# anihcsam/OpenGaussian

Hardware: AMD Instinct MI355X
Metric: fwd+bwd Mpix/s at 1080p, 1M Gaussians (RGB+6-D ins_feat); k-means it/s (higher is better)
Workload: dtype f32; 1 GPU; S1M-1080p RGB(SH3)+depth+alpha (all grads) + 6-ch ins_feat (grad to ins_feat) fwd+bwd, ONE fused 9-channel pass; gaussians=1000000, width=1920, height=1080, views_cycled=8, parallelism=single

## Files before the change

### include/ogs_raster.h

```cpp
#ifndef OGS_RASTER_H
#define OGS_RASTER_H

#include <stddef.h>
#include <stdint.h>

#ifdef __cplusplus
extern "C" {
#endif

#define OGS_OK 0
#define OGS_ERR_INVALID_ARG (-1)
#define OGS_ERR_HIP (-2)
#define OGS_ERR_UNSUPPORTED (-3)
#define OGS_ERR_SCRATCH_TOO_SMALL (-4)
#define OGS_ERR_DEVICE (-5)

#define OGS_TILE 16
#define OGS_MAX_CHANNELS 12

typedef struct OgsRasterFwdArgs {
    int32_t P;
    int32_t W, H;
    int32_t C;
    int32_t sh_degree;
    int32_t sh_coeffs;
    float tanfovx, tanfovy;
    float scale_modifier;
    int32_t prefiltered;
    int32_t debug;
    const float* bg;
    const float* means3D;
    const float* colors_precomp;
    const float* shs;
    const float* opacities;
    const float* scales;
    const float* rotations;
    const float* cov3D_precomp;
    const float* viewmatrix;
    const float* projmatrix;
    const float* campos;
    float* out_color;
    float* out_depth;
    float* out_alpha;
    int32_t* radii;
    void* geom_buffer;
    void* geom_tmp;
    void* image_buffer;
    uint32_t* point_list;
    void* binning_tmp;
    void* sorted_rec;
    void* quad_list;
    const int32_t* group_ids;
    int32_t num_groups;
    int32_t full_binning;
    void* bwd_clear;
    size_t bwd_clear_bytes;
} OgsRasterFwdArgs;

typedef struct OgsRasterBwdArgs {
    int32_t P, W, H, C, sh_degree, sh_coeffs;
    float tanfovx, tanfovy, scale_modifier;
    int32_t debug;
    int32_t num_rendered;
    int32_t geom_channels;
    const float* bg;
    const float* means3D;
    const float* colors_precomp;
    const float* shs;
    const float* opacities;
    const float* scales;
    const float* rotations;
    const float* cov3D_precomp;
    const float* viewmatrix;
    const float* projmatrix;
    const float* campos;
    const int32_t* radii;
    const float* out_alpha;
    const float* dL_dcolor;
    const float* dL_ddepth;
    const float* dL_dalpha;
    const void* geom_buffer;
    const void* image_buffer;
    const uint32_t* point_list;
    const void* sorted_rec;
    const void* quad_list;
    void* bwd_tmp;
    float* dL_dmeans2D;
    float* dL_dcolors;
    float* dL_dopacity;
    float* dL_dmeans3D;
    float* dL_dcov3D;
    float* dL_dsh;
    float* dL_dscales;
    float* dL_drotations;
    int32_t num_groups;
    float* dL_dsh_rgb;
    int32_t bwd_tmp_is_clear;
} OgsRasterBwdArgs;

int ogs_version(void);
const char* ogs_last_error(void);

int ogs_check_async_status(void);

size_t ogs_raster_geom_bytes(int32_t P, int32_t C);
size_t ogs_raster_geom_tmp_bytes(int32_t P);
size_t ogs_raster_image_bytes(int32_t W, int32_t H);
size_t ogs_raster_image_bytes_grouped(int32_t W, int32_t H, int32_t num_groups);
size_t ogs_raster_binning_tmp_bytes(int64_t num_rendered, int32_t W, int32_t H);
size_t ogs_raster_backward_tmp_bytes(int32_t P);
size_t ogs_raster_sorted_bytes(int64_t num_rendered, int32_t C);
size_t ogs_raster_quad_list_bytes(int64_t num_rendered);

int ogs_raster_forward_geometry(const OgsRasterFwdArgs* args, void* stream, int64_t* num_rendered_host);

int ogs_raster_forward_render(const OgsRasterFwdArgs* args, int64_t num_rendered, void* stream);

int ogs_raster_read_num_rendered_async(const OgsRasterFwdArgs* args, void* stream, uint32_t* host_pinned);
int ogs_raster_forward_render_deferred(const OgsRasterFwdArgs* args, int64_t capacity, void* stream);

int ogs_raster_read_num_emitted(const OgsRasterFwdArgs* args, void* stream, uint32_t* host);

size_t ogs_raster_tiny_max_points(void);
int ogs_raster_forward_tiny(const OgsRasterFwdArgs* args, void* stream);

size_t ogs_raster_tile_sort_capacity(int32_t level);

int ogs_raster_forward_reblend(const OgsRasterFwdArgs* args, void* stream);

int ogs_raster_compact_kept(int32_t W, int32_t H, int32_t C, const void* image_buffer, const void* sorted_rec,
                            const void* quad_list, void* new_image_buffer, void* new_sorted_rec, void* new_quad_list,
                            void* stream);

typedef struct OgsGroupStatsArgs {
    const int32_t* labels;
    int32_t num_labels;
    float alpha_threshold;
    float* max_alpha;
    int64_t* count;
    float* feat_sum;
    void* stats_tmp;
} OgsGroupStatsArgs;

size_t ogs_raster_stats_image_bytes(int32_t W, int32_t H, int32_t num_groups);
size_t ogs_raster_stats_tmp_bytes(int32_t num_groups, int32_t num_labels, int32_t C);
int ogs_raster_forward_group_stats(const OgsRasterFwdArgs* args, const OgsGroupStatsArgs* stats, int64_t num_rendered,
                                   void* stream);

int ogs_raster_backward(const OgsRasterBwdArgs* args, void* stream);

int ogs_mark_visible(int32_t P, const float* means3D, const float* viewmatrix, const float* projmatrix,
                     uint8_t* present, void* stream);

int ogs_sh_grad_from_views(int32_t P, int32_t V, int32_t sh_degree, int32_t sh_coeffs, const float* means3D,
                           const float* campos, const float* dL_drgb, float* dL_dsh, void* stream);

int ogs_raster_export_binning(const OgsRasterFwdArgs* args, int64_t num_rendered, uint64_t* keys_out,
                              uint32_t* ranges_out, uint32_t* n_contrib_out, void* stream);

int ogs_prof_enable(int on);
int ogs_prof_filter(const char* prefix);
int ogs_prof_collect(char* buf, size_t n);

int ogs_selftest_wave_fold16(const float* in, float* out, void* stream);
int ogs_selftest_mfma_rank1(const float* w, const float* f, const float* acc0, int32_t steps, float* out_mfma, float* out_fma,
                            void* stream);
int ogs_selftest_tile_order(const uint32_t* ranges, int64_t vtiles, uint32_t* order, void* stream);
size_t ogs_selftest_radix_tmp_bytes(int64_t n);
int ogs_selftest_radix_sort(uint32_t* keys0, uint32_t* vals0, uint32_t* keys1, uint32_t* vals1, int64_t n, int32_t key_bits,
                            int32_t variant, int32_t items, const uint32_t* n_dev, void* tmp, int32_t* result_buffer,
                            void* stream);

#ifdef __cplusplus
}
#endif
#endif
```

### opengaussian_amd/_lib.py

```python
from __future__ import annotations

import ctypes as C
import os

_HERE = os.path.dirname(os.path.abspath(__file__))
LIB_PATH = os.environ.get("OGS_LIB_PATH") or os.path.join(_HERE, "lib", "libogs_hip.so")

_f32p = C.POINTER(C.c_float)
_vp = C.c_void_p


class OgsRasterFwdArgs(C.Structure):
    _fields_ = [
        ("P", C.c_int32), ("W", C.c_int32), ("H", C.c_int32), ("C", C.c_int32),
        ("sh_degree", C.c_int32), ("sh_coeffs", C.c_int32),
        ("tanfovx", C.c_float), ("tanfovy", C.c_float), ("scale_modifier", C.c_float),
        ("prefiltered", C.c_int32), ("debug", C.c_int32),
        ("bg", _vp), ("means3D", _vp), ("colors_precomp", _vp), ("shs", _vp), ("opacities", _vp),
        ("scales", _vp), ("rotations", _vp), ("cov3D_precomp", _vp),
        ("viewmatrix", _vp), ("projmatrix", _vp), ("campos", _vp),
        ("out_color", _vp), ("out_depth", _vp), ("out_alpha", _vp), ("radii", _vp),
        ("geom_buffer", _vp), ("geom_tmp", _vp), ("image_buffer", _vp), ("point_list", _vp),
        ("binning_tmp", _vp), ("sorted_rec", _vp), ("quad_list", _vp), ("group_ids", _vp), ("num_groups", C.c_int32),
        ("full_binning", C.c_int32),
        ("bwd_clear", _vp), ("bwd_clear_bytes", C.c_size_t),
    ]


class OgsRasterBwdArgs(C.Structure):
    _fields_ = [
        ("P", C.c_int32), ("W", C.c_int32), ("H", C.c_int32), ("C", C.c_int32),
        ("sh_degree", C.c_int32), ("sh_coeffs", C.c_int32),
        ("tanfovx", C.c_float), ("tanfovy", C.c_float), ("scale_modifier", C.c_float),
        ("debug", C.c_int32), ("num_rendered", C.c_int32), ("geom_channels", C.c_int32),
        ("bg", _vp), ("means3D", _vp), ("colors_precomp", _vp), ("shs", _vp), ("opacities", _vp),
        ("scales", _vp), ("rotations", _vp), ("cov3D_precomp", _vp),
        ("viewmatrix", _vp), ("projmatrix", _vp), ("campos", _vp),
        ("radii", _vp), ("out_alpha", _vp), ("dL_dcolor", _vp), ("dL_ddepth", _vp), ("dL_dalpha", _vp),
        ("geom_buffer", _vp), ("image_buffer", _vp), ("point_list", _vp), ("sorted_rec", _vp), ("quad_list", _vp), ("bwd_tmp", _vp),
        ("dL_dmeans2D", _vp), ("dL_dcolors", _vp), ("dL_dopacity", _vp), ("dL_dmeans3D", _vp),
        ("dL_dcov3D", _vp), ("dL_dsh", _vp), ("dL_dscales", _vp), ("dL_drotations", _vp), ("num_groups", C.c_int32), ("dL_dsh_rgb", _vp),
        ("bwd_tmp_is_clear", C.c_int32),
    ]


class OgsAdamTensor(C.Structure):
    _fields_ = [("param", _vp), ("grad", _vp), ("exp_avg", _vp), ("exp_avg_sq", _vp), ("numel", C.c_int64),
                ("lr", C.c_double), ("step", C.c_int64)]


class OgsRowTensor(C.Structure):
    _fields_ = [("src", _vp), ("dst", _vp), ("width", C.c_int32), ("zero_new", C.c_int32)]


class OgsDensifyArgs(C.Structure):
    _fields_ = [("N", C.c_int32), ("grad_accum", _vp), ("denom", _vp), ("scaling", _vp), ("opacity", _vp),
                ("max_grad", C.c_float), ("min_opacity", C.c_float), ("extent", C.c_float), ("percent_dense", C.c_float),
                ("prune_world_size", C.c_int32)]


class OgsGroupStatsArgs(C.Structure):
    _fields_ = [("labels", _vp), ("num_labels", C.c_int32), ("alpha_threshold", C.c_float), ("max_alpha", _vp),
                ("count", _vp), ("feat_sum", _vp), ("stats_tmp", _vp)]


class OgsLabelMapArgs(C.Structure):
    _fields_ = [("labels", _vp), ("num_labels", C.c_int32), ("out_label", _vp), ("out_weight", _vp), ("out_second", _vp),
                ("out_alpha", _vp)]


class OgsLabelVotesArgs(C.Structure):
    _fields_ = [("pixel_labels", _vp), ("num_labels", C.c_int32), ("rows", _vp), ("num_rows", C.c_int32), ("votes", _vp)]


class OgsFeatureVotesArgs(C.Structure):
    _fields_ = [("features", _vp), ("num_channels", C.c_int32), ("valid", _vp), ("rows", _vp), ("num_rows", C.c_int32),
                ("votes", _vp)]


class OgsFeatureMapArgs(C.Structure):
    _fields_ = [("features", _vp), ("num_channels", C.c_int32), ("rows", _vp), ("num_rows", C.c_int32),
                ("channels_last", C.c_int32), ("out_map", _vp), ("out_alpha", _vp)]


class OgsRawModel(C.Structure):
    _fields_ = [("features_dc", _vp), ("features_rest", _vp), ("scaling", _vp), ("rotation", _vp), ("opacity", _vp)]


class OgsRawModelGrads(C.Structure):
    _fields_ = [("features_dc", _vp), ("features_rest", _vp), ("scaling", _vp), ("rotation", _vp), ("opacity", _vp)]


SIGNATURES = {
    "ogs_version": (C.c_int, []),
    "ogs_last_error": (C.c_char_p, []),
    "ogs_raster_geom_bytes": (C.c_size_t, [C.c_int32, C.c_int32]),
    "ogs_raster_geom_tmp_bytes": (C.c_size_t, [C.c_int32]),
    "ogs_raster_image_bytes": (C.c_size_t, [C.c_int32, C.c_int32]),
    "ogs_raster_image_bytes_grouped": (C.c_size_t, [C.c_int32, C.c_int32, C.c_int32]),
    "ogs_raster_binning_tmp_bytes": (C.c_size_t, [C.c_int64, C.c_int32, C.c_int32]),
    "ogs_raster_backward_tmp_bytes": (C.c_size_t, [C.c_int32]),
    "ogs_raster_sorted_bytes": (C.c_size_t, [C.c_int64, C.c_int32]),
    "ogs_raster_quad_list_bytes": (C.c_size_t, [C.c_int64]),
    "ogs_raster_forward_geometry": (C.c_int, [C.POINTER(OgsRasterFwdArgs), _vp, C.POINTER(C.c_int64)]),
    "ogs_raster_forward_render": (C.c_int, [C.POINTER(OgsRasterFwdArgs), C.c_int64, _vp]),
    "ogs_raster_read_num_rendered_async": (C.c_int, [C.POINTER(OgsRasterFwdArgs), _vp, _vp]),
    "ogs_raster_forward_render_deferred": (C.c_int, [C.POINTER(OgsRasterFwdArgs), C.c_int64, _vp]),
    "ogs_raster_read_num_emitted": (C.c_int, [C.POINTER(OgsRasterFwdArgs), _vp, C.POINTER(C.c_uint32)]),
    "ogs_raster_stats_image_bytes": (C.c_size_t, [C.c_int32, C.c_int32, C.c_int32]),
    "ogs_raster_stats_tmp_bytes": (C.c_size_t, [C.c_int32, C.c_int32, C.c_int32]),
    "ogs_raster_forward_group_stats": (C.c_int, [C.POINTER(OgsRasterFwdArgs), C.POINTER(OgsGroupStatsArgs), C.c_int64, _vp]),
    "ogs_raster_backward": (C.c_int, [C.POINTER(OgsRasterBwdArgs), _vp]),
    "ogs_raster_tiny_max_points": (C.c_size_t, []),
    "ogs_raster_tile_sort_capacity": (C.c_size_t, [C.c_int32]),
    "ogs_raster_forward_tiny": (C.c_int, [C.POINTER(OgsRasterFwdArgs), _vp]),
    "ogs_raster_forward_reblend": (C.c_int, [C.POINTER(OgsRasterFwdArgs), _vp]),
    "ogs_raster_compact_kept": (C.c_int, [C.c_int32, C.c_int32, C.c_int32, _vp, _vp, _vp, _vp, _vp, _vp, _vp]),
    "ogs_mark_visible": (C.c_int, [C.c_int32, _vp, _vp, _vp, _vp, _vp]),
    "ogs_sh_grad_from_views": (C.c_int, [C.c_int32, C.c_int32, C.c_int32, C.c_int32, _vp, _vp, _vp, _vp, _vp]),
    "ogs_raster_export_binning": (C.c_int, [C.POINTER(OgsRasterFwdArgs), C.c_int64, _vp, _vp, _vp, _vp]),
    "ogs_selftest_wave_fold16": (C.c_int, [_vp, _vp, _vp]),
    "ogs_selftest_mfma_rank1": (C.c_int, [_vp, _vp, _vp, C.c_int32, _vp, _vp, _vp]),
    "ogs_selftest_tile_order": (C.c_int, [_vp, C.c_int64, _vp, _vp]),
    "ogs_selftest_radix_tmp_bytes": (C.c_size_t, [C.c_int64]),
    "ogs_selftest_radix_sort": (C.c_int, [_vp, _vp, _vp, _vp, C.c_int64, C.c_int32, C.c_int32, C.c_int32, _vp, _vp, _vp, _vp]),
    "ogs_raster_forward_geometry_raw": (C.c_int, [C.POINTER(OgsRasterFwdArgs), C.POINTER(OgsRawModel), _vp,
                                                  C.POINTER(C.c_int64)]),
    "ogs_raster_forward_tiny_raw": (C.c_int, [C.POINTER(OgsRasterFwdArgs), C.POINTER(OgsRawModel), _vp]),
    "ogs_raster_backward_raw": (C.c_int, [C.POINTER(OgsRasterBwdArgs), C.POINTER(OgsRawModel), C.POINTER(OgsRawModelGrads), _vp]),
    "ogs_model_activate": (C.c_int, [C.c_int32, C.c_int32, C.POINTER(OgsRawModel), _vp, _vp, _vp, _vp, _vp]),
    "ogs_check_async_status": (C.c_int, []),
    "ogs_prof_enable": (C.c_int, [C.c_int]),
    "ogs_prof_filter": (C.c_int, [C.c_char_p]),
    "ogs_prof_collect": (C.c_int, [C.c_char_p, C.c_size_t]),
    "ogs_kmeans_tmp_bytes": (C.c_size_t, [C.c_int64, C.c_int32, C.c_int32]),
    "ogs_kmeans_lloyd": (C.c_int, [_vp, C.c_int64, C.c_int32, _vp, C.c_int32, C.c_int32, C.c_int32, C.c_int32,
                                   _vp, C.c_int64, _vp, _vp]),
    "ogs_kmeans_assign": (C.c_int, [_vp, C.c_int64, C.c_int32, _vp, C.c_int32, _vp, C.c_int64, _vp]),
    "ogs_mask_feature_sums": (C.c_int, [_vp, _vp, _vp, C.c_int32, C.c_int32, C.c_int64, C.c_int32, _vp, _vp]),
    "ogs_mask_feature_sqdev": (C.c_int, [_vp, _vp, _vp, _vp, C.c_int32, C.c_int32, C.c_int64, _vp, _vp]),
    "ogs_mask_feature_sums_backward": (C.c_int, [_vp, _vp, _vp, _vp, _vp, C.c_int32, C.c_int32, C.c_int64, _vp, _vp, _vp]),
    "ogs_mask_cohesion": (C.c_int, [_vp, _vp, _vp, C.c_int32, C.c_int32, C.c_int64, _vp, _vp]),
    "ogs_mask_cohesion_backward": (C.c_int, [_vp, _vp, _vp, _vp, C.c_int32, C.c_int32, C.c_int64, _vp, _vp, _vp]),
    "ogs_label_feature_sums": (C.c_int, [_vp, _vp, _vp, C.c_int32, C.c_int32, C.c_int64, C.c_int32, _vp, _vp]),
    "ogs_label_feature_sqdev": (C.c_int, [_vp, _vp, _vp, _vp, C.c_int32, C.c_int32, C.c_int64, _vp, _vp]),
    "ogs_label_feature_sums_backward": (C.c_int, [_vp, _vp, _vp, _vp, _vp, C.c_int32, C.c_int32, C.c_int64, _vp, _vp, _vp]),
    "ogs_label_cohesion": (C.c_int, [_vp, _vp, _vp, C.c_int32, C.c_int32, C.c_int64, _vp, _vp]),
    "ogs_label_cohesion_backward": (C.c_int, [_vp, _vp, _vp, _vp, C.c_int32, C.c_int32, C.c_int64, _vp, _vp, _vp]),
    "ogs_separation_loss": (C.c_int, [_vp, C.c_int32, C.c_int32, C.c_int32, _vp, _vp, _vp, _vp]),
    "ogs_adam_step": (C.c_int, [C.POINTER(OgsAdamTensor), C.c_int32, C.c_double, C.c_double, C.c_double, _vp]),
    "ogs_rows_gather": (C.c_int, [C.POINTER(OgsRowTensor), C.c_int32, _vp, _vp, C.c_int64, _vp]),
    "ogs_densify_tmp_bytes": (C.c_size_t, [C.c_int32]),
    "ogs_densify_plan": (C.c_int, [C.POINTER(OgsDensifyArgs), _vp, C.POINTER(C.c_uint32), _vp]),
    "ogs_densify_map": (C.c_int, [C.c_int32, _vp, _vp, _vp, _vp, _vp]),
    "ogs_densify_split_children": (C.c_int, [C.c_int64, _vp, _vp, _vp, _vp, _vp, _vp, _vp, _vp, _vp, _vp]),
    "ogs_densify_stats": (C.c_int, [C.c_int32, _vp, C.c_int32, _vp, _vp, _vp, _vp, _vp, _vp]),
    "ogs_kmeans_accumulate": (C.c_int, [_vp, C.c_int64, C.c_int32, _vp, C.c_int32, C.c_int32, _vp, _vp, _vp]),
    "ogs_kmeans_update": (C.c_int, [_vp, C.c_int32, C.c_int32, C.c_int32, _vp, _vp, _vp]),
    "ogs_kmeans_gather": (C.c_int, [_vp, _vp, C.c_int64, C.c_int32, C.c_int32, _vp, _vp]),
    "ogs_refine_wave_table_capacity": (C.c_size_t, []),
    "ogs_refine_wave_max_pixels": (C.c_size_t, []),
    "ogs_refine_block_scratch_words": (C.c_size_t, [C.c_int32]),
    "ogs_refine_visibility": (C.c_int, [C.c_int32, _vp, _vp, _vp, _vp, C.c_int32, C.c_int32, C.c_float, C.c_float, _vp,
                                        C.c_float, C.c_float, _vp, _vp]),
    "ogs_refine_footprint_labels": (C.c_int, [C.c_int32, _vp, _vp, C.c_int32, C.c_int32, C.c_int32, _vp, C.c_int32, _vp, _vp,
                                              _vp]),
    "ogs_refine_footprint_labels_block": (C.c_int, [C.c_int32, _vp, _vp, C.c_int32, C.c_int32, C.c_int32, _vp, C.c_int32, _vp,
                                                    _vp, _vp, _vp]),
    "ogs_refine_vote": (C.c_int, [C.c_int64, C.c_int32, _vp, _vp, _vp]),
    "ogs_refine_expand": (C.c_int, [C.c_int32, _vp, _vp, _vp, _vp, C.c_int32, C.c_int32, C.c_int32, _vp, C.c_int32, _vp, _vp,
                                    C.c_int32, _vp]),
    "ogs_refine_finalize": (C.c_int, [C.c_int64, C.c_int32, _vp, _vp, _vp, C.c_int32, C.c_float, _vp, _vp]),
    "ogs_loss_photometric_tmp_bytes": (C.c_size_t, [C.c_int32, C.c_int32, C.c_int32]),
    "ogs_loss_photometric_forward": (C.c_int, [_vp, _vp, C.c_int32, C.c_int32, C.c_int32, C.c_float, _vp, _vp, _vp]),
    "ogs_loss_photometric_backward": (C.c_int, [_vp, _vp, _vp, _vp, _vp, C.c_float, C.c_int32, C.c_int32, C.c_int32, _vp,
                                                _vp]),
    "ogs_loss_masked_tmp_bytes": (C.c_size_t, []),
    "ogs_loss_masked_forward": (C.c_int, [_vp, _vp, _vp, _vp, C.c_int32, C.c_int32, C.c_int32, C.c_int64, _vp, _vp, _vp]),
    "ogs_loss_masked_backward": (C.c_int, [_vp, _vp, _vp, _vp, C.c_int32, C.c_int32, C.c_int32, C.c_int64, _vp, _vp, _vp,
                                           _vp]),
    "ogs_knn_tile_points": (C.c_size_t, []),
    "ogs_knn_group_ksum": (C.c_int, [C.c_int64, _vp, C.c_int32, _vp, _vp, _vp, _vp, _vp, _vp]),
    "ogs_knn_box_points": (C.c_size_t, []),
    "ogs_knn_max_k": (C.c_size_t, []),
    "ogs_knn_neighbors_tmp_bytes": (C.c_size_t, [C.c_int64]),
    "ogs_knn_neighbors": (C.c_int, [C.c_int64, _vp, C.c_int32, C.c_int32, _vp, _vp, _vp, C.c_size_t, _vp]),
    "ogs_knn_aggregate": (C.c_int, [C.c_int64, C.c_int32, C.c_int64, C.c_int32, _vp, _vp, _vp, _vp, _vp]),
    "ogs_knn_transpose_chunk": (C.c_size_t, []),
    "ogs_knn_transpose_tmp_bytes": (C.c_size_t, [C.c_int64, C.c_int32, C.c_int64]),
    "ogs_knn_transpose": (C.c_int, [C.c_int64, C.c_int32, C.c_int64, _vp, _vp, _vp, _vp, C.c_size_t, _vp]),
    "ogs_knn_aggregate_t_tmp_bytes": (C.c_size_t, [C.c_int64, C.c_int32, C.c_int64, C.c_int32]),
    "ogs_knn_aggregate_t": (C.c_int, [C.c_int64, C.c_int32, C.c_int64, C.c_int32, _vp, _vp, _vp, _vp, _vp, _vp, C.c_size_t,
                                      _vp]),
    "ogs_knn_edge_dots": (C.c_int, [C.c_int64, C.c_int32, C.c_int64, C.c_int32, _vp, _vp, _vp, _vp, _vp]),
    "ogs_knn_smoothness_fwd_tmp_bytes": (C.c_size_t, [C.c_int64]),
    "ogs_knn_smoothness_fwd": (C.c_int, [C.c_int64, C.c_int32, C.c_int32, _vp, _vp, _vp, _vp, _vp, _vp, C.c_size_t, _vp]),
    "ogs_knn_smoothness_bwd_tmp_bytes": (C.c_size_t, [C.c_int64, C.c_int32, C.c_int32]),
    "ogs_knn_smoothness_bwd": (C.c_int, [C.c_int64, C.c_int32, C.c_int32, _vp, _vp, _vp, _vp, _vp, _vp, _vp, _vp, _vp,
                                         C.c_size_t, _vp]),
    "ogs_kmeans_wide_row_tile": (C.c_size_t, []),
    "ogs_kmeans_wide_centre_tile": (C.c_size_t, []),
    "ogs_kmeans_wide_dim_step": (C.c_size_t, []),
    "ogs_kmeans_wide_stage": (C.c_size_t, []),
    "ogs_kmeans_wide_max_dim": (C.c_size_t, []),
    "ogs_kmeans_wide_max_k": (C.c_size_t, []),
    "ogs_kmeans_wide_tmp_bytes": (C.c_size_t, [C.c_int64, C.c_int32, C.c_int32]),
    "ogs_kmeans_wide_assign": (C.c_int, [_vp, C.c_int64, C.c_int32, _vp, C.c_int32, C.c_int32, _vp, _vp, _vp, C.c_size_t, _vp]),
    "ogs_kmeans_wide_update": (C.c_int, [_vp, _vp, C.c_int64, C.c_int32, _vp, C.c_int32, C.c_int32, _vp, _vp, _vp, C.c_size_t,
                                         _vp]),
    "ogs_kmeans_wide_inertia": (C.c_int, [_vp, _vp, C.c_int64, _vp, _vp, C.c_size_t, _vp]),
    "ogs_kmeans_wide_lloyd": (C.c_int, [_vp, _vp, C.c_int64, C.c_int32, _vp, C.c_int32, C.c_int32, C.c_int32, _vp, _vp, _vp, _vp,
                                        _vp, C.c_size_t, _vp]),
    "ogs_query_max_leaves": (C.c_size_t, []),
    "ogs_query_max_top": (C.c_size_t, []),
    "ogs_query_max_classes": (C.c_size_t, []),
    "ogs_query_confusion_block": (C.c_size_t, []),
    "ogs_query_split_block": (C.c_size_t, []),
    "ogs_query_split_tmp_bytes": (C.c_size_t, [C.c_int64, C.c_int32]),
    "ogs_query_select": (C.c_int, [C.c_int32, C.c_int32, C.c_int32, _vp, _vp, _vp, _vp, C.c_int32, C.c_float, C.c_float,
                                   C.c_int32, _vp, _vp, _vp, _vp]),
    "ogs_query_classify": (C.c_int, [C.c_int64, _vp, C.c_int32, C.c_int32, _vp, _vp, _vp, _vp]),
    "ogs_query_confusion": (C.c_int, [C.c_int64, _vp, _vp, _vp, C.c_int32, _vp, _vp]),
    "ogs_query_split_count": (C.c_int, [C.c_int64, _vp, C.c_int32, _vp, _vp, C.c_int32, _vp, _vp]),
    "ogs_query_split_scan": (C.c_int, [C.c_int64, C.c_int32, _vp, _vp, _vp, _vp, _vp]),
    "ogs_query_split_scatter": (C.c_int, [C.c_int64, _vp, C.c_int32, _vp, _vp, C.c_int32, _vp, _vp, _vp, C.c_int64, _vp]),
    "ogs_raster_label_map": (C.c_int, [C.POINTER(OgsRasterFwdArgs), C.POINTER(OgsLabelMapArgs), _vp]),
    "ogs_label_map_tile_capacity": (C.c_size_t, []),
    "ogs_raster_label_votes": (C.c_int, [C.POINTER(OgsRasterFwdArgs), C.POINTER(OgsLabelVotesArgs), _vp]),
    "ogs_label_votes_quadrant_capacity": (C.c_size_t, []),
    "ogs_label_votes_fold_columns": (C.c_size_t, []),
    "ogs_raster_feature_votes": (C.c_int, [C.POINTER(OgsRasterFwdArgs), C.POINTER(OgsFeatureVotesArgs), _vp]),
    "ogs_feature_votes_fold_columns": (C.c_size_t, []),
    "ogs_feature_votes_block_columns": (C.c_size_t, []),
    "ogs_raster_feature_map": (C.c_int, [C.POINTER(OgsRasterFwdArgs), C.POINTER(OgsFeatureMapArgs), _vp]),
    "ogs_feature_map_fold_columns": (C.c_size_t, []),
    "ogs_feature_map_block_columns": (C.c_size_t, []),
}

_lib = None


class OgsError(RuntimeError):
    pass


def lib() -> C.CDLL:
    global _lib
    if _lib is None:
        if not os.path.exists(LIB_PATH):
            raise OgsError(f"{LIB_PATH} not found -- build it with `python -m opengaussian_amd.build` "
                           "(the product path has no CPU fallback)")
        import torch
        l = C.CDLL(LIB_PATH)
        for name, (res, args) in SIGNATURES.items():
            fn = getattr(l, name)
            fn.restype = res
            fn.argtypes = args
        _lib = l
    return _lib


def check(rc: int, what: str):
    if rc != 0:
        raise OgsError(f"{what} failed (code {rc}): {lib().ogs_last_error().decode()}")


def prof_filter(prefix: str):
    check(lib().ogs_prof_filter(prefix.encode()), "ogs_prof_filter")


def prof_enable(mode):
    check(lib().ogs_prof_enable(int(mode)), "ogs_prof_enable")


def prof_collect() -> dict:
    import json
    buf = C.create_string_buffer(1 << 16)
    check(lib().ogs_prof_collect(buf, len(buf)), "ogs_prof_collect")
    return json.loads(buf.value.decode())


def ptr(t):
    return None if t is None else t.data_ptr()
```

### opengaussian_amd/csrc/binning.hip

```cpp
#include <stdlib.h>
#include <string.h>

#include "ogs_common.h"

namespace ogs {

namespace {

constexpr size_t kSweepHeaderWords = 4 * 256 + 4 + 60;
constexpr int kScanItems = 8;
constexpr int kScanTile = kBlock * kScanItems;

__device__ __forceinline__ uint32_t wave_inclusive_scan(uint32_t v) {
#pragma unroll
    for (int d = 1; d < kWave; d <<= 1) {
        uint32_t t = __shfl_up(v, d, kWave);
        if (lane_id() >= d) v += t;
    }
    return v;
}

__device__ __forceinline__ uint32_t block_exclusive_scan(uint32_t v, uint32_t& total, uint32_t* wave_sums ) {
    const int wave = threadIdx.x >> 6;
    const uint32_t inc = wave_inclusive_scan(v);
    if (lane_id() == kWave - 1) wave_sums[wave] = inc;
    __syncthreads();
    uint32_t base = 0, tot = 0;
#pragma unroll
    for (int w = 0; w < kBlock / kWave; ++w) {
        const uint32_t s = wave_sums[w];
        if (w < wave) base += s;
        tot += s;
    }
    total = tot;
    __syncthreads();
    return base + inc - v;
}

__device__ __forceinline__ void load_items(const uint32_t* __restrict__ in, const uint32_t* __restrict__ gather,
                                           int64_t base, int64_t n, uint32_t item[kScanItems]) {
#pragma unroll
    for (int i = 0; i < kScanItems; ++i) {
        const int64_t idx = base + i;
        uint32_t v = 0;
        if (idx < n) v = gather ? in[gather[idx]] : in[idx];
        item[i] = v;
    }
}

__global__ __launch_bounds__(kBlock) void scan_reduce_kernel(const uint32_t* __restrict__ in,
                                                             const uint32_t* __restrict__ gather, int64_t n,
                                                             uint32_t* __restrict__ partials, const uint32_t* __restrict__ n_dev) {
    __shared__ uint32_t wave_sums[4];
    if (n_dev) n = min(n, (int64_t)*n_dev);
    const int64_t base = (int64_t)blockIdx.x * kScanTile + (int64_t)threadIdx.x * kScanItems;
    uint32_t item[kScanItems];
    load_items(in, gather, base, n, item);
    uint32_t s = 0;
#pragma unroll
    for (int i = 0; i < kScanItems; ++i) s += item[i];
    uint32_t total;
    block_exclusive_scan(s, total, wave_sums);
    if (threadIdx.x == 0) partials[blockIdx.x] = total;
}

template <bool SUM_PARTIALS>
__global__ __launch_bounds__(kBlock) void scan_apply_kernel(const uint32_t* __restrict__ in,
                                                            const uint32_t* __restrict__ gather,
                                                            uint32_t* __restrict__ out, int64_t n,
                                                            const uint32_t* __restrict__ partial_offsets,
                                                            uint32_t* __restrict__ total_out, const uint32_t* __restrict__ n_dev) {
    __shared__ uint32_t wave_sums[4];
    if (n_dev) n = min(n, (int64_t)*n_dev);
    const int64_t base = (int64_t)blockIdx.x * kScanTile + (int64_t)threadIdx.x * kScanItems;
    uint32_t item[kScanItems];
    load_items(in, gather, base, n, item);
    uint32_t s = 0;
#pragma unroll
    for (int i = 0; i < kScanItems; ++i) s += item[i];
    uint32_t block_base = 0;
    if (SUM_PARTIALS) {
        uint32_t acc = 0;
        for (uint32_t j = threadIdx.x; j < blockIdx.x; j += kBlock) acc += partial_offsets[j];
        uint32_t tot;
        block_exclusive_scan(acc, tot, wave_sums);
        block_base = tot;
    } else if (partial_offsets) {
        block_base = partial_offsets[blockIdx.x];
    }
    uint32_t total;
    uint32_t run = block_exclusive_scan(s, total, wave_sums) + block_base;
#pragma unroll
    for (int i = 0; i < kScanItems; ++i) {
        const int64_t idx = base + i;
        if (idx < n) out[idx] = run;
        run += item[i];
    }
    if (total_out && threadIdx.x == 0) {
        if (SUM_PARTIALS) { if (blockIdx.x == gridDim.x - 1) *total_out = block_base + total; }
        else if (partial_offsets == nullptr) *total_out = total;
    }
}

__global__ void scan_total_kernel(const uint32_t* __restrict__ in, const uint32_t* __restrict__ gather,
                                  const uint32_t* __restrict__ out, int64_t n, uint32_t* __restrict__ total_out,
                                  const uint32_t* __restrict__ n_dev) {
    if (threadIdx.x == 0 && blockIdx.x == 0) {
        if (n_dev) n = min(n, (int64_t)*n_dev);
        if (n <= 0) { *total_out = 0u; return; }
        const uint32_t last = gather ? in[gather[n - 1]] : in[n - 1];
        *total_out = out[n - 1] + last;
    }
}

inline int scan_blocks(int64_t n) { return (int)((n + kScanTile - 1) / kScanTile); }
constexpr int kFlatScanBlocks = 16384;

template <int ITEMS>
__global__ __launch_bounds__(kBlock) void radix_hist_kernel(const uint32_t* __restrict__ keys, int64_t n_cap,
                                                            const uint32_t* __restrict__ n_dev, int shift,
                                                            int bits, uint32_t* __restrict__ hist, int nblocks, bool drop) {
    __shared__ uint32_t h[256];
    const int64_t n = n_dev ? min((int64_t)*n_dev, n_cap) : n_cap;
    const int ndig = 1 << bits;
    const uint32_t mask = ndig - 1;
    h[threadIdx.x] = 0;
    __syncthreads();
    const int64_t base = (int64_t)blockIdx.x * (kBlock * ITEMS);
#pragma unroll
    for (int i = 0; i < ITEMS; ++i) {
        const int64_t idx = base + i * kBlock + threadIdx.x;
        if (idx < n) {
            const uint32_t k = keys[idx];
            if (!(drop && k == kDropKey)) atomicAdd(&h[(k >> shift) & mask], 1u);
        }
    }
    __syncthreads();
    if ((int)threadIdx.x < ndig) hist[(size_t)threadIdx.x * nblocks + blockIdx.x] = h[threadIdx.x];
}

__global__ __launch_bounds__(kBlock) void radix_rowscan_kernel(uint32_t* __restrict__ hist, int nblocks,
                                                               uint32_t* __restrict__ row_total) {
    __shared__ uint32_t wave_sums[4];
    uint32_t* row = hist + (size_t)blockIdx.x * nblocks;
    uint32_t carry = 0;
    for (int base = 0; base < nblocks; base += kScanTile) {
        uint32_t item[kScanItems];
        const int b0 = base + (int)threadIdx.x * kScanItems;
        uint32_t sum = 0;
#pragma unroll
        for (int i = 0; i < kScanItems; ++i) {
            item[i] = (b0 + i < nblocks) ? row[b0 + i] : 0u;
            sum += item[i];
        }
        uint32_t total;
        uint32_t run = carry + block_exclusive_scan(sum, total, wave_sums);
#pragma unroll
        for (int i = 0; i < kScanItems; ++i) {
            if (b0 + i < nblocks) row[b0 + i] = run;
            run += item[i];
        }
        carry += total;
    }
    if (threadIdx.x == 0) row_total[blockIdx.x] = carry;
}

template <int ITEMS>
__global__ __launch_bounds__(kBlock) void radix_scatter_kernel(const uint32_t* __restrict__ keys_in,
                                                               const uint32_t* __restrict__ vals_in,
                                                               uint32_t* __restrict__ keys_out,
                                                               uint32_t* __restrict__ vals_out, int64_t n_cap,
                                                               const uint32_t* __restrict__ n_dev, int shift,
                                                               int bits, const uint32_t* __restrict__ offsets,
                                                               const uint32_t* __restrict__ row_total,
                                                               int nblocks, bool drop, uint32_t* __restrict__ kept_out) {
    __shared__ uint32_t wave_hist_s[kBlock / kWave][256];
    __shared__ uint32_t scan_sums[4];
    __shared__ uint32_t dig_start[256], glob_base[256];
    __shared__ uint32_t stage_k[kBlock * ITEMS], stage_v[kBlock * ITEMS];
    volatile uint32_t(*wave_hist)[256] = wave_hist_s;
    const int64_t n = n_dev ? min((int64_t)*n_dev, n_cap) : n_cap;
    const int ndig = 1 << bits;
    const uint32_t mask = ndig - 1;
    const int tid = threadIdx.x, lane = tid & 63, wave = tid >> 6;
#pragma unroll
    for (int w = 0; w < kBlock / kWave; ++w) wave_hist_s[w][tid] = 0;
    __syncthreads();

    const int64_t base = (int64_t)blockIdx.x * (kBlock * ITEMS) + (int64_t)wave * (ITEMS * kWave);
    uint32_t key[ITEMS], val[ITEMS], rank[ITEMS];
#pragma unroll
    for (int i = 0; i < ITEMS; ++i) {
        const int64_t idx = base + i * kWave + lane;
        const bool valid = idx < n;
        key[i] = valid ? keys_in[idx] : 0xFFFFFFFFu;
        val[i] = valid ? vals_in[idx] : 0u;
    }
    const uint64_t lt_mask = (1ull << lane) - 1ull;
#pragma unroll
    for (int i = 0; i < ITEMS; ++i) {
        const int64_t idx = base + i * kWave + lane;
        const bool valid = drop ? key[i] != kDropKey : idx < n;
        const uint32_t d = (key[i] >> shift) & mask;
        uint64_t peers = __ballot(valid);
        for (int b = 0; b < bits; ++b) {
            const bool bit = (d >> b) & 1u;
            const uint64_t m = __ballot(bit);
            peers &= bit ? m : ~m;
        }
        const uint32_t r = __popcll(peers & lt_mask);
        const uint32_t cnt = __popcll(peers);
        uint32_t pre = 0;
        if (valid) pre = wave_hist[wave][d];
        __builtin_amdgcn_wave_barrier();
        if (valid && r == 0) wave_hist[wave][d] = pre + cnt;
        __builtin_amdgcn_wave_barrier();
        rank[i] = pre + r;
    }
    __syncthreads();
    uint32_t run_len = 0;
    if (tid < ndig) {
#pragma unroll
        for (int w = 0; w < kBlock / kWave; ++w) {
            const uint32_t t = wave_hist_s[w][tid];
            wave_hist_s[w][tid] = run_len;
            run_len += t;
        }
    }
    uint32_t n_valid;
    const uint32_t local_start = block_exclusive_scan(run_len, n_valid, scan_sums);
    uint32_t dummy_total;
    const uint32_t digit_base = block_exclusive_scan(tid < ndig ? row_total[tid] : 0u, dummy_total, scan_sums);
    if (kept_out != nullptr && blockIdx.x == 0 && tid == 0) *kept_out = dummy_total;
    if (tid < ndig) {
        dig_start[tid] = local_start;
        glob_base[tid] = digit_base + offsets[(size_t)tid * nblocks + blockIdx.x] - local_start;
    }
    __syncthreads();
#pragma unroll
    for (int i = 0; i < ITEMS; ++i) {
        const int64_t idx = base + i * kWave + lane;
        if (drop ? key[i] != kDropKey : idx < n) {
            const uint32_t d = (key[i] >> shift) & mask;
            const uint32_t lp = dig_start[d] + wave_hist_s[wave][d] + rank[i];
            stage_k[lp] = key[i];
            stage_v[lp] = val[i];
        }
    }
    __syncthreads();
    for (uint32_t j = tid; j < n_valid; j += kBlock) {
        const uint32_t k = stage_k[j];
        const uint32_t pos = glob_base[(k >> shift) & mask] + j;
        keys_out[pos] = k;
        vals_out[pos] = stage_v[j];
    }
}

constexpr uint32_t kStatAgg = 1u << 30, kStatInc = 2u << 30, kStatMask = (1u << 30) - 1u;
constexpr int kSpinLimit = 1 << 22;
constexpr int kLookBack = 8;
constexpr int kHistAllBlocks = 256;

struct RadixPlanDev { int npass; int shift[4]; int bits[4]; };

__global__ __launch_bounds__(kBlock) void radix_hist_all_kernel(const uint32_t* __restrict__ keys, int64_t n_cap,
                                                                const uint32_t* __restrict__ n_dev, RadixPlanDev plan,
                                                                uint32_t* __restrict__ ghist , bool drop) {
    __shared__ uint32_t h[4][256];
    const int64_t n = n_dev ? min((int64_t)*n_dev, n_cap) : n_cap;
#pragma unroll
    for (int p = 0; p < 4; ++p) h[p][threadIdx.x] = 0;
    __syncthreads();
    for (int64_t idx = (int64_t)blockIdx.x * kBlock + threadIdx.x; idx < n; idx += (int64_t)gridDim.x * kBlock) {
        const uint32_t k = keys[idx];
        if (drop && k == kDropKey) continue;
#pragma unroll
        for (int p = 0; p < 4; ++p)
            if (p < plan.npass) atomicAdd(&h[p][(k >> plan.shift[p]) & ((1u << plan.bits[p]) - 1u)], 1u);
    }
    __syncthreads();
#pragma unroll
    for (int p = 0; p < 4; ++p)
        if (p < plan.npass && h[p][threadIdx.x] != 0) atomicAdd(&ghist[p * 256 + threadIdx.x], h[p][threadIdx.x]);
}

template <int ITEMS>
__global__ __launch_bounds__(kBlock) void radix_onesweep_kernel(const uint32_t* __restrict__ keys_in,
                                                                const uint32_t* __restrict__ vals_in,
                                                                uint32_t* __restrict__ keys_out,
                                                                uint32_t* __restrict__ vals_out, int64_t n_cap,
                                                                const uint32_t* __restrict__ n_dev, int shift, int bits,
                                                                const uint32_t* __restrict__ ghist ,
                                                                uint32_t* __restrict__ status ,
                                                                uint32_t* __restrict__ ticket ,
                                                                uint32_t* __restrict__ status_word ,
                                                                int spin_limit, bool drop,
                                                                uint32_t* __restrict__ kept_out) {
    __shared__ uint32_t wave_hist_s[kBlock / kWave][256];
    __shared__ uint32_t scan_sums[4];
    __shared__ uint32_t dig_start[256], glob_base[256];
    __shared__ uint32_t stage_k[kBlock * ITEMS], stage_v[kBlock * ITEMS];
    __shared__ uint32_t s_ticket;
    volatile uint32_t(*wave_hist)[256] = wave_hist_s;
    const int64_t n = n_dev ? min((int64_t)*n_dev, n_cap) : n_cap;
    const int ndig = 1 << bits;
    const uint32_t mask = ndig - 1;
    const int tid = threadIdx.x, lane = tid & 63, wave = tid >> 6;
    if (tid == 0) s_ticket = atomicAdd(ticket, 1u);
#pragma unroll
    for (int w = 0; w < kBlock / kWave; ++w) wave_hist_s[w][tid] = 0;
    __syncthreads();
    const uint32_t tile = s_ticket;
    if ((int64_t)tile * (kBlock * ITEMS) >= n) {
        if (kept_out != nullptr && tile == 0 && tid == 0) *kept_out = 0u;
        return;
    }

    const int64_t base = (int64_t)tile * (kBlock * ITEMS) + (int64_t)wave * (ITEMS * kWave);
    uint32_t key[ITEMS], val[ITEMS], rank[ITEMS];
#pragma unroll
    for (int i = 0; i < ITEMS; ++i) {
        const int64_t idx = base + i * kWave + lane;
        const bool valid = idx < n;
        key[i] = valid ? keys_in[idx] : 0xFFFFFFFFu;
        val[i] = valid ? vals_in[idx] : 0u;
    }
    const uint64_t lt_mask = (1ull << lane) - 1ull;
#pragma unroll
    for (int i = 0; i < ITEMS; ++i) {
        const int64_t idx = base + i * kWave + lane;
        const bool valid = drop ? key[i] != kDropKey : idx < n;
        const uint32_t d = (key[i] >> shift) & mask;
        uint64_t peers = __ballot(valid);
        for (int b = 0; b < bits; ++b) {
            const bool bit = (d >> b) & 1u;
            const uint64_t m = __ballot(bit);
            peers &= bit ? m : ~m;
        }
        const uint32_t r = __popcll(peers & lt_mask);
        const uint32_t cnt = __popcll(peers);
        uint32_t pre = 0;
        if (valid) pre = wave_hist[wave][d];
        __builtin_amdgcn_wave_barrier();
        if (valid && r == 0) wave_hist[wave][d] = pre + cnt;
        __builtin_amdgcn_wave_barrier();
        rank[i] = pre + r;
    }
    __syncthreads();
    uint32_t run_len = 0;
    if (tid < ndig) {
#pragma unroll
        for (int w = 0; w < kBlock / kWave; ++w) {
            const uint32_t t = wave_hist_s[w][tid];
            wave_hist_s[w][tid] = run_len;
            run_len += t;
        }
        __hip_atomic_store(&status[(size_t)tile * 256 + tid], (tile == 0 ? kStatInc : kStatAgg) | run_len,
                           __ATOMIC_RELAXED, __HIP_MEMORY_SCOPE_AGENT);
    }
    uint32_t n_valid;
    const uint32_t local_start = block_exclusive_scan(run_len, n_valid, scan_sums);
    uint32_t dummy_total;
    const uint32_t digit_base = block_exclusive_scan(tid < ndig ? ghist[tid] : 0u, dummy_total, scan_sums);
    if (kept_out != nullptr && tile == 0 && tid == 0) *kept_out = dummy_total;
    uint32_t before = 0;
    if (tid < ndig && tile > 0) {
        int64_t pb = (int64_t)tile - 1;
        int spins = 0;
        bool done = false;
        while (!done) {
            uint32_t sw[kLookBack];
#pragma unroll
            for (int k = 0; k < kLookBack; ++k)
                sw[k] = pb - k >= 0 ? __hip_atomic_load(&status[(size_t)(pb - k) * 256 + tid], __ATOMIC_RELAXED, __HIP_MEMORY_SCOPE_AGENT)
                                    : kStatInc;
            int used = 0;
#pragma unroll
            for (int k = 0; k < kLookBack; ++k) {
                if (done || used != k) continue;
                const uint32_t flag = sw[k] & ~kStatMask;
                if (flag == 0u) continue;
                before += sw[k] & kStatMask;
                used = k + 1;
                done = flag == kStatInc;
            }
            pb -= used;
            if (!done && used < kLookBack) {
                if (++spins > spin_limit) {
                    __hip_atomic_fetch_or(status_word, kAsyncRadixSpin, __ATOMIC_RELAXED, __HIP_MEMORY_SCOPE_SYSTEM);
                    break;
                }
                __builtin_amdgcn_s_sleep(1);
            }
        }
        __hip_atomic_store(&status[(size_t)tile * 256 + tid], kStatInc | ((before + run_len) & kStatMask),
                           __ATOMIC_RELAXED, __HIP_MEMORY_SCOPE_AGENT);
    }
    if (tid < ndig) {
        dig_start[tid] = local_start;
        glob_base[tid] = digit_base + before - local_start;
    }
    __syncthreads();
#pragma unroll
    for (int i = 0; i < ITEMS; ++i) {
        const int64_t idx = base + i * kWave + lane;
        if (drop ? key[i] != kDropKey : idx < n) {
            const uint32_t d = (key[i] >> shift) & mask;
            const uint32_t lp = dig_start[d] + wave_hist_s[wave][d] + rank[i];
            stage_k[lp] = key[i];
            stage_v[lp] = val[i];
        }
    }
    __syncthreads();
    for (uint32_t j = tid; j < n_valid; j += kBlock) {
        const uint32_t k = stage_k[j];
        const uint32_t pos = glob_base[(k >> shift) & mask] + j;
        if ((int64_t)pos < n) {
            keys_out[pos] = k;
            vals_out[pos] = stage_v[j];
        }
    }
}

constexpr int kRangeItems = 4;
__global__ __launch_bounds__(kBlock) void tile_ranges_kernel(const uint32_t* __restrict__ tile_keys, int64_t D_cap,
                                                             const uint32_t* __restrict__ n_dev,
                                                             uint2* __restrict__ ranges) {
    const int64_t D = n_dev ? min((int64_t)*n_dev, D_cap) : D_cap;
    const int64_t i0 = ((int64_t)blockIdx.x * kBlock + threadIdx.x) * kRangeItems;
    if (i0 >= D) return;
    uint32_t k[kRangeItems];
    if (i0 + kRangeItems <= D) {
        const uint4 v = *reinterpret_cast<const uint4*>(tile_keys + i0);
        k[0] = v.x; k[1] = v.y; k[2] = v.z; k[3] = v.w;
    } else {
#pragma unroll
        for (int j = 0; j < kRangeItems; ++j) k[j] = i0 + j < D ? tile_keys[i0 + j] : 0u;
    }
    uint32_t prev = i0 > 0 ? tile_keys[i0 - 1] : 0u;
#pragma unroll
    for (int j = 0; j < kRangeItems; ++j) {
        const int64_t i = i0 + j;
        if (i < D) {
            const uint32_t cur = k[j];
            if (i == 0) {
                ranges[cur].x = 0;
            } else if (prev != cur) {
                ranges[prev].y = (uint32_t)i;
                ranges[cur].x = (uint32_t)i;
            }
            if (i == D - 1) ranges[cur].y = (uint32_t)D;
            prev = cur;
        }
    }
}

constexpr int kTileSortWaves = kBlock / kWave;
struct TileSortLds {
    uint32_t hist[kTileSortWaves][256];
    uint32_t dig_start[256];
    uint32_t base[256];
    uint32_t scan_sums[4];
    uint32_t red[2];
    uint2 range[kTileSortWaves];
    uint32_t kv[2 * kTileSortCap];
};
typedef __attribute__((address_space(3))) volatile uint32_t LdsWord;
typedef __attribute__((address_space(3))) unsigned long long LdsMask;
__device__ __forceinline__ LdsWord* lds_words(uint32_t* p) { return (LdsWord*)p; }
__device__ __forceinline__ LdsMask* wave_masks(TileSortLds& sm, int wave) { return (LdsMask*)(sm.kv + wave * 2 * kWaveSortCap); }

__device__ __forceinline__ void wave_rank_clear(LdsWord* hist, LdsMask* masks) {
    const int lane = threadIdx.x & (kWave - 1);
#pragma unroll
    for (int j = 0; j < 4; ++j) {
        hist[lane + j * kWave] = 0u;
        __hip_atomic_store(&masks[lane + j * kWave], 0ull, __ATOMIC_SEQ_CST, __HIP_MEMORY_SCOPE_WAVEFRONT);
    }
    __builtin_amdgcn_wave_barrier();
}

__device__ __forceinline__ void wave_rank(LdsWord* hist, LdsMask* masks, const uint32_t (&key)[kTileSortItems],
                                          uint32_t (&rank)[kTileSortItems], int ipl, int first, int m, int shift,
                                          uint32_t mask) {
    const int lane = threadIdx.x & (kWave - 1);
    const unsigned long long me = 1ull << lane;
#pragma unroll
    for (int i = 0; i < kTileSortItems; ++i) {
        if (i >= ipl) continue;
        const bool valid = first + i * kWave + lane < m;
        const uint32_t d = (key[i] >> shift) & mask;
        if (valid) __hip_atomic_fetch_or(&masks[d], me, __ATOMIC_SEQ_CST, __HIP_MEMORY_SCOPE_WAVEFRONT);
        __builtin_amdgcn_wave_barrier();
        const unsigned long long peers =
            valid ? __hip_atomic_load(&masks[d], __ATOMIC_SEQ_CST, __HIP_MEMORY_SCOPE_WAVEFRONT) : 0ull;
        const uint32_t r = __builtin_amdgcn_mbcnt_hi((uint32_t)(peers >> 32), __builtin_amdgcn_mbcnt_lo((uint32_t)peers, 0u));
        uint32_t pre = 0;
        if (valid) pre = hist[d];
        __builtin_amdgcn_wave_barrier();
        if (valid && r == 0) {
            hist[d] = pre + (uint32_t)__popcll(peers);
            __hip_atomic_store(&masks[d], 0ull, __ATOMIC_SEQ_CST, __HIP_MEMORY_SCOPE_WAVEFRONT);
        }
        __builtin_amdgcn_wave_barrier();
        rank[i] = pre + r;
    }
}

__device__ __forceinline__ void load_items(const uint32_t* __restrict__ list, const uint32_t* __restrict__ depth_keys,
                                           uint32_t (&key)[kTileSortItems], uint32_t (&val)[kTileSortItems], int ipl, int first,
                                           int m) {
#pragma unroll
    for (int i = 0; i < kTileSortItems; ++i) {
        if (i >= ipl) continue;
        val[i] = list[min(first + i * kWave, m - 1)];
    }
#pragma unroll
    for (int i = 0; i < kTileSortItems; ++i) {
        if (i >= ipl) continue;
        key[i] = depth_keys[val[i] & kGidMask];
    }
}

__device__ __forceinline__ uint32_t tile_sort_rank(TileSortLds& sm, const uint32_t (&key)[kTileSortItems],
                                                   uint32_t (&rank)[kTileSortItems], int ipl, int chunk, int m, int shift,
                                                   uint32_t mask) {
    const int tid = threadIdx.x, wave = tid >> 6;
    LdsWord* hist = lds_words(sm.hist[wave]);
    LdsMask* masks = wave_masks(sm, wave);
    wave_rank_clear(hist, masks);
    wave_rank(hist, masks, key, rank, ipl, wave * chunk, m, shift, mask);
    __syncthreads();
    uint32_t run_len = 0;
#pragma unroll
    for (int w = 0; w < kTileSortWaves; ++w) {
        const uint32_t t = sm.hist[w][tid];
        sm.hist[w][tid] = run_len;
        run_len += t;
    }
    uint32_t total;
    sm.dig_start[tid] = block_exclusive_scan(run_len, total, sm.scan_sums);
    __syncthreads();
    return run_len;
}

__device__ __forceinline__ void wave_sort_list(TileSortLds& sm, uint32_t* __restrict__ seg, int n,
                                               const uint32_t* __restrict__ depth_keys) {
    const int lane = threadIdx.x & (kWave - 1), wave = threadIdx.x >> 6;
    LdsWord* wk = lds_words(sm.kv + wave * 2 * kWaveSortCap);
    LdsWord* wv = wk + kWaveSortCap;
    LdsWord* hist = lds_words(sm.hist[wave]);
    LdsMask* masks = wave_masks(sm, wave);
    uint32_t key[kTileSortItems], val[kTileSortItems], rank[kTileSortItems];
    const int ipl = (n + kWave - 1) / kWave;
    load_items(seg, depth_keys, key, val, ipl, lane, n);
    uint32_t k_and = 0xFFFFFFFFu, k_or = 0u;
#pragma unroll
    for (int i = 0; i < kTileSortItems; ++i) {
        if (i >= ipl) continue;
        k_and &= key[i];
        k_or |= key[i];
    }
#pragma unroll
    for (int d = 32; d >= 1; d >>= 1) {
        k_and &= (uint32_t)__shfl_xor((int)k_and, d, kWave);
        k_or |= (uint32_t)__shfl_xor((int)k_or, d, kWave);
    }
    const uint32_t diff = (uint32_t)__builtin_amdgcn_readfirstlane((int)(k_and ^ k_or));
    if (diff == 0u) return;
    const int lo = __builtin_ctz(diff), hi = 31 - __builtin_clz(diff);
    const int npass = (hi - lo + 8) / 8;
    const int per = (hi - lo + npass) / npass;
    for (int p = 0; p < npass; ++p) {
        const int shift = lo + p * per, bits = min(per, hi + 1 - shift);
        const uint32_t mask = (1u << bits) - 1u;
        wave_rank_clear(hist, masks);
        wave_rank(hist, masks, key, rank, ipl, 0, n, shift, mask);
        uint32_t c[4], sum = 0;
#pragma unroll
        for (int j = 0; j < 4; ++j) { c[j] = hist[4 * lane + j]; sum += c[j]; }
        uint32_t run = wave_inclusive_scan(sum) - sum;
#pragma unroll
        for (int j = 0; j < 4; ++j) { hist[4 * lane + j] = run; run += c[j]; }
        __builtin_amdgcn_wave_barrier();
#pragma unroll
        for (int i = 0; i < kTileSortItems; ++i) {
            if (i >= ipl) continue;
            rank[i] += hist[(key[i] >> shift) & mask];
        }
#pragma unroll
        for (int i = 0; i < kTileSortItems; ++i) {
            if (i >= ipl) continue;
            if (i * kWave + lane < n) {
                wk[rank[i]] = key[i];
                wv[rank[i]] = val[i];
            }
        }
        __builtin_amdgcn_wave_barrier();
        if (p + 1 < npass) {
#pragma unroll
            for (int i = 0; i < kTileSortItems; ++i) {
                if (i >= ipl) continue;
                const int e = min(i * kWave + lane, n - 1);
                key[i] = wk[e];
                val[i] = wv[e];
            }
            __builtin_amdgcn_wave_barrier();
        }
    }
    for (int j = lane; j < n; j += kWave) seg[j] = wv[j];
}

__device__ __forceinline__ void block_sort_list(TileSortLds& sm, uint32_t* __restrict__ seg, uint32_t* __restrict__ alt, int n,
                                                const uint32_t* __restrict__ depth_keys) {
    const int tid = threadIdx.x, lane = tid & 63, wave = tid >> 6;
    const bool in_lds = n <= kTileSortCap;
    uint32_t key[kTileSortItems], val[kTileSortItems], rank[kTileSortItems];
    __syncthreads();
    if (tid < 2) sm.red[tid] = tid == 0 ? 0xFFFFFFFFu : 0u;
    uint32_t k_and = 0xFFFFFFFFu, k_or = 0u;
    const int ipl0 = (min(n, kTileSortCap) + kBlock - 1) / kBlock, chunk0 = ipl0 * kWave;
    if (in_lds) {
        load_items(seg, depth_keys, key, val, ipl0, wave * chunk0 + lane, n);
#pragma unroll
        for (int i = 0; i < kTileSortItems; ++i) {
            if (i >= ipl0) continue;
            k_and &= key[i];
            k_or |= key[i];
        }
    } else {
        for (int j = tid; j < n; j += kBlock) {
            const uint32_t k = depth_keys[seg[j] & kGidMask];
            k_and &= k;
            k_or |= k;
        }
    }
#pragma unroll
    for (int d = 32; d >= 1; d >>= 1) {
        k_and &= (uint32_t)__shfl_xor((int)k_and, d, kWave);
        k_or |= (uint32_t)__shfl_xor((int)k_or, d, kWave);
    }
    __syncthreads();
    if (lane == 0) { atomicAnd(&sm.red[0], k_and); atomicOr(&sm.red[1], k_or); }
    __syncthreads();
    const uint32_t diff = sm.red[0] ^ sm.red[1];
    if (diff == 0u) return;
    const int lo = __builtin_ctz(diff), hi = 31 - __builtin_clz(diff);
    const int npass = (hi - lo + 8) / 8;
    const int per = (hi - lo + npass) / npass;
    uint32_t* const sk = sm.kv;
    uint32_t* const sv = sm.kv + kTileSortCap;

    if (in_lds) {
        for (int p = 0; p < npass; ++p) {
            const int shift = lo + p * per, bits = min(per, hi + 1 - shift);
            const uint32_t mask = (1u << bits) - 1u;
            tile_sort_rank(sm, key, rank, ipl0, chunk0, n, shift, mask);
#pragma unroll
            for (int i = 0; i < kTileSortItems; ++i) {
                if (i >= ipl0) continue;
                const uint32_t d = (key[i] >> shift) & mask;
                rank[i] += sm.dig_start[d] + sm.hist[wave][d];
            }
#pragma unroll
            for (int i = 0; i < kTileSortItems; ++i) {
                if (i >= ipl0) continue;
                if (wave * chunk0 + i * kWave + lane < n) {
                    sk[rank[i]] = key[i];
                    sv[rank[i]] = val[i];
                }
            }
            __syncthreads();
            if (p + 1 < npass) {
#pragma unroll
                for (int i = 0; i < kTileSortItems; ++i) {
                    if (i >= ipl0) continue;
                    const int e = min(wave * chunk0 + i * kWave + lane, n - 1);
                    key[i] = sk[e];
                    val[i] = sv[e];
                }
                __syncthreads();
            }
        }
        for (int j = tid; j < n; j += kBlock) seg[j] = sv[j];
        return;
    }

    for (int p = 0; p < npass; ++p) {
        const int shift = lo + p * per, bits = min(per, hi + 1 - shift);
        const uint32_t mask = (1u << bits) - 1u;
        const uint32_t* __restrict__ src = (p & 1) ? alt : seg;
        uint32_t* __restrict__ dst = (p & 1) ? seg : alt;
        sm.base[tid] = 0u;
        __syncthreads();
        for (int j = tid; j < n; j += kBlock) atomicAdd(&sm.base[(depth_keys[src[j] & kGidMask] >> shift) & mask], 1u);
        __syncthreads();
        uint32_t total;
        const uint32_t start = block_exclusive_scan(sm.base[tid], total, sm.scan_sums);
        sm.base[tid] = start;
        for (int c0 = 0; c0 < n; c0 += kTileSortCap) {
            const int m = min(kTileSortCap, n - c0);
            const int ipl = (m + kBlock - 1) / kBlock, chunk = ipl * kWave;
            load_items(src + c0, depth_keys, key, val, ipl, wave * chunk + lane, m);
            const uint32_t cnt = tile_sort_rank(sm, key, rank, ipl, chunk, m, shift, mask);
#pragma unroll
            for (int i = 0; i < kTileSortItems; ++i) {
                if (i >= ipl) continue;
                if (wave * chunk + i * kWave + lane < m) {
                    const uint32_t d = (key[i] >> shift) & mask;
                    dst[sm.base[d] + sm.hist[wave][d] + rank[i]] = val[i];
                }
            }
            __syncthreads();
            sm.base[tid] += cnt;
        }
        __syncthreads();
    }
    if (npass & 1) {
        for (int j = tid; j < n; j += kBlock) seg[j] = alt[j];
    }
}

__global__ __launch_bounds__(kBlock) void tile_depth_sort_kernel(const uint2* __restrict__ ranges, int tiles,
                                                                 const uint32_t* __restrict__ tile_order,
                                                                 uint32_t* __restrict__ point_list,
                                                                 const uint32_t* __restrict__ depth_keys,
                                                                 uint32_t* __restrict__ scratch) {
    __shared__ TileSortLds sm;
    const int wave = threadIdx.x >> 6;
    if (threadIdx.x < kTileSortWaves) {
        const int b = blockIdx.x * kTileSortWaves + threadIdx.x;
        sm.range[threadIdx.x] = b < tiles ? ranges[tile_order ? tile_order[b] : (uint32_t)b] : make_uint2(0u, 0u);
    }
    __syncthreads();
    const uint32_t x = (uint32_t)__builtin_amdgcn_readfirstlane((int)sm.range[wave].x);
    const int n = __builtin_amdgcn_readfirstlane((int)(sm.range[wave].y - sm.range[wave].x));
    if (n >= 2 && n <= kWaveSortCap) wave_sort_list(sm, point_list + x, n, depth_keys);
#pragma unroll 1
    for (int w = 0; w < kTileSortWaves; ++w) {
        const uint32_t xw = (uint32_t)__builtin_amdgcn_readfirstlane((int)sm.range[w].x);
        const int nw = __builtin_amdgcn_readfirstlane((int)(sm.range[w].y - sm.range[w].x));
        if (nw > kWaveSortCap) block_sort_list(sm, point_list + xw, scratch + xw, nw, depth_keys);
    }
}

__global__ __launch_bounds__(kBlock) void export_keys_kernel(const uint2* __restrict__ ranges,
                                                             const uint32_t* __restrict__ point_list,
                                                             const float4* __restrict__ rec, int recv4,
                                                             uint64_t* __restrict__ keys_out) {
    const uint32_t tile = blockIdx.x;
    const uint2 r = ranges[tile];
    for (uint32_t i = r.x + threadIdx.x; i < r.y; i += kBlock) {
        const uint32_t gid = point_list[i] & kGidMask;
        const uint32_t bits = __float_as_uint(rec[(size_t)gid * recv4].z);
        keys_out[i] = ((uint64_t)tile << 32) | bits;
    }
}

}

size_t scan_tmp_bytes(int64_t n) {
    size_t total = 0;
    int64_t m = n;
    while (true) {
        const int nb = scan_blocks(m);
        if (nb <= 1) break;
        total += align_up((size_t)nb * sizeof(uint32_t));
        m = nb;
    }
    return total + kAlign;
}

size_t sort_tmp_bytes(int64_t n) {
    const int64_t hist = (int64_t)256 * sort_blocks_for(n > 0 ? n : 1);
    const size_t legacy = align_up((size_t)hist * sizeof(uint32_t)) + align_up(256 * sizeof(uint32_t)) + scan_tmp_bytes(hist);
    const int64_t tiles4 = ((n > 0 ? n : 1) + kBlock * 4 - 1) / (kBlock * 4);
    const size_t sweep = align_up(kSweepHeaderWords * sizeof(uint32_t)) + 4 * align_up((size_t)256 * tiles4 * sizeof(uint32_t));
    return legacy > sweep ? legacy : sweep;
}

static int sweep_items_for(int64_t n, int forced) {
    if (forced == 4 || forced == 16) return forced;
    return n <= (int64_t)(256 << 10) ? 4 : 16;
}

bool radix_onesweep_enabled(int64_t n) {
    static const int forced = [] {
        const char* e = getenv("OGS_RADIX");
        return !e ? 0 : strcmp(e, "legacy") == 0 ? 1 : strcmp(e, "sweep") == 0 ? 2 : 0;
    }();
    if (forced == 1 || n >= (int64_t)kStatMask) return false;
    return forced == 2 || n <= (int64_t)(256 << 10);
}

namespace {
struct SweepTmp {
    uint32_t* ghist;
    uint32_t* ticket;
    uint32_t* status[4];
    size_t zero_bytes;
    static SweepTmp carve(void* tmp, int64_t n, int npass, int items_forced) {
        SweepTmp t;
        char* p = static_cast<char*>(tmp);
        t.ghist = reinterpret_cast<uint32_t*>(p);
        t.ticket = t.ghist + 4 * 256;
        const int items = sweep_items_for(n, items_forced);
        const int64_t tiles = ((n > 0 ? n : 1) + (int64_t)kBlock * items - 1) / ((int64_t)kBlock * items);
        const size_t table = align_up((size_t)256 * tiles * sizeof(uint32_t));
        char* q = p + align_up(kSweepHeaderWords * sizeof(uint32_t));
        for (int i = 0; i < 4; ++i) t.status[i] = reinterpret_cast<uint32_t*>(q + (size_t)i * table);
        t.zero_bytes = align_up(kSweepHeaderWords * sizeof(uint32_t)) + (size_t)npass * table;
        return t;
    }
};
}

int radix_sort_begin(const uint32_t* keys, int64_t n, const uint32_t* n_dev, int npass, const int* shifts, const int* bits,
                     void* tmp, hipStream_t stream, int debug, bool drop, int items) {
    if (n <= 0) return OGS_OK;
    if (npass < 1 || npass > 4) { set_error("radix_sort_begin: npass=%d out of range", npass); return OGS_ERR_INVALID_ARG; }
    const SweepTmp t = SweepTmp::carve(tmp, n, npass, items);
    OGS_HIP_CHECK(hipMemsetAsync(tmp, 0, t.zero_bytes, stream));
    RadixPlanDev plan{};
    plan.npass = npass;
    for (int i = 0; i < npass; ++i) {
        if (bits[i] < 1 || bits[i] > 8) { set_error("radix_sort_begin: bits=%d out of range", bits[i]); return OGS_ERR_INVALID_ARG; }
        plan.shift[i] = shifts[i];
        plan.bits[i] = bits[i];
    }
    const int64_t want = (n + kBlock * 16 - 1) / (kBlock * 16);
    const int grid = (int)(want < 1 ? 1 : (want > kHistAllBlocks ? kHistAllBlocks : want));
    OGS_LAUNCH(radix_hist_all_kernel, dim3(grid), dim3(kBlock), 0, stream, keys, n, n_dev, plan, t.ghist, drop);
    OGS_LAUNCH_CHECK(debug, stream);
    return OGS_OK;
}

int radix_sort_pass(int pass, int npass, const uint32_t* keys_in, const uint32_t* vals_in, uint32_t* keys_out, uint32_t* vals_out,
                    int64_t n, int shift, int bits, void* tmp, hipStream_t stream, int debug, const uint32_t* n_dev, bool drop,
                    uint32_t* kept_out, int items_forced, int spin_limit) {
    if (n <= 0) return OGS_OK;
    const SweepTmp t = SweepTmp::carve(tmp, n, npass, items_forced);
    const int items = sweep_items_for(n, items_forced);
    const int nb = (int)((n + (int64_t)kBlock * items - 1) / ((int64_t)kBlock * items));
    uint32_t* status_word = async_status_word();
    if (!status_word) return OGS_ERR_HIP;
    if (spin_limit < 0) spin_limit = kSpinLimit;
    if (items == 4) {
        OGS_LAUNCH(radix_onesweep_kernel<4>, dim3(nb), dim3(kBlock), 0, stream, keys_in, vals_in, keys_out, vals_out, n, n_dev,
                   shift, bits, (const uint32_t*)(t.ghist + pass * 256), t.status[pass], t.ticket + pass, status_word, spin_limit,
                   drop, kept_out);
    } else {
        OGS_LAUNCH(radix_onesweep_kernel<16>, dim3(nb), dim3(kBlock), 0, stream, keys_in, vals_in, keys_out, vals_out, n, n_dev,
                   shift, bits, (const uint32_t*)(t.ghist + pass * 256), t.status[pass], t.ticket + pass, status_word, spin_limit,
                   drop, kept_out);
    }
    OGS_LAUNCH_CHECK(debug, stream);
    return OGS_OK;
}

int exclusive_scan_u32(const uint32_t* in, const uint32_t* gather, uint32_t* out, int64_t n, uint32_t* total,
                       void* tmp, hipStream_t stream, int debug, const uint32_t* n_dev) {
    if (n <= 0) {
        if (total) OGS_HIP_CHECK(hipMemsetAsync(total, 0, sizeof(uint32_t), stream));
        return OGS_OK;
    }
    const int nb = scan_blocks(n);
    if (nb == 1) {
        OGS_LAUNCH(scan_apply_kernel<false>, dim3(1), dim3(kBlock), 0, stream, in, gather, out, n,
                           (const uint32_t*)nullptr, total, n_dev);
        OGS_LAUNCH_CHECK(debug, stream);
        return OGS_OK;
    }
    uint32_t* partials = static_cast<uint32_t*>(tmp);
    void* next_tmp = static_cast<char*>(tmp) + align_up((size_t)nb * sizeof(uint32_t));
    OGS_LAUNCH(scan_reduce_kernel, dim3(nb), dim3(kBlock), 0, stream, in, gather, n, partials, n_dev);
    OGS_LAUNCH_CHECK(debug, stream);
    if (nb <= kFlatScanBlocks) {
        OGS_LAUNCH(scan_apply_kernel<true>, dim3(nb), dim3(kBlock), 0, stream, in, gather, out, n,
                           (const uint32_t*)partials, total, n_dev);
        OGS_LAUNCH_CHECK(debug, stream);
        return OGS_OK;
    }
    int rc = exclusive_scan_u32(partials, nullptr, partials, nb, nullptr, next_tmp, stream, debug, nullptr);
    if (rc != OGS_OK) return rc;
    OGS_LAUNCH(scan_apply_kernel<false>, dim3(nb), dim3(kBlock), 0, stream, in, gather, out, n,
                       (const uint32_t*)partials, (uint32_t*)nullptr, n_dev);
    OGS_LAUNCH_CHECK(debug, stream);
    if (total) {
        if (in == out) { set_error("exclusive_scan_u32: total with in-place scan unsupported"); return OGS_ERR_INVALID_ARG; }
        OGS_LAUNCH(scan_total_kernel, dim3(1), dim3(64), 0, stream, in, gather, (const uint32_t*)out, n, total, n_dev);
        OGS_LAUNCH_CHECK(debug, stream);
    }
    return OGS_OK;
}

int radix_pass(const uint32_t* keys_in, const uint32_t* vals_in, uint32_t* keys_out, uint32_t* vals_out, int64_t n,
               int shift, int bits, void* tmp, hipStream_t stream, int debug, const uint32_t* n_dev, bool drop,
               uint32_t* kept_out) {
    if (n <= 0) return OGS_OK;
    if (bits < 1 || bits > 8) { set_error("radix_pass: bits=%d out of range", bits); return OGS_ERR_INVALID_ARG; }
    const int items = sort_items_for(n);
    const int nb = sort_blocks_for(n);
    const int ndig = 1 << bits;
    uint32_t* hist = static_cast<uint32_t*>(tmp);
    uint32_t* row_total = reinterpret_cast<uint32_t*>(static_cast<char*>(tmp) + align_up((size_t)256 * nb * sizeof(uint32_t)));
    if (items == 4) {
        OGS_LAUNCH(radix_hist_kernel<4>, dim3(nb), dim3(kBlock), 0, stream, keys_in, n, n_dev, shift, bits, hist, nb, drop);
    } else {
        OGS_LAUNCH(radix_hist_kernel<8>, dim3(nb), dim3(kBlock), 0, stream, keys_in, n, n_dev, shift, bits, hist, nb, drop);
    }
    OGS_LAUNCH_CHECK(debug, stream);
    OGS_LAUNCH(radix_rowscan_kernel, dim3(ndig), dim3(kBlock), 0, stream, hist, nb, row_total);
    OGS_LAUNCH_CHECK(debug, stream);
    if (items == 4) {
        OGS_LAUNCH(radix_scatter_kernel<4>, dim3(nb), dim3(kBlock), 0, stream, keys_in, vals_in, keys_out, vals_out, n, n_dev,
                   shift, bits, (const uint32_t*)hist, (const uint32_t*)row_total, nb, drop, kept_out);
    } else {
        OGS_LAUNCH(radix_scatter_kernel<8>, dim3(nb), dim3(kBlock), 0, stream, keys_in, vals_in, keys_out, vals_out, n, n_dev,
                   shift, bits, (const uint32_t*)hist, (const uint32_t*)row_total, nb, drop, kept_out);
    }
    OGS_LAUNCH_CHECK(debug, stream);
    return OGS_OK;
}

int launch_tile_ranges(const uint32_t* tile_keys_sorted, int64_t D, uint2* ranges, int64_t tiles, hipStream_t s,
                       int debug, const uint32_t* n_dev, bool already_zeroed) {
    if (!already_zeroed) OGS_HIP_CHECK(hipMemsetAsync(ranges, 0, (size_t)tiles * sizeof(uint2), s));
    if (D <= 0) return OGS_OK;
    const int grid = (int)((D + (int64_t)kBlock * kRangeItems - 1) / ((int64_t)kBlock * kRangeItems));
    OGS_LAUNCH(tile_ranges_kernel, dim3(grid), dim3(kBlock), 0, s, tile_keys_sorted, D, n_dev, ranges);
    OGS_LAUNCH_CHECK(debug, s);
    return OGS_OK;
}

int launch_tile_depth_sort(const uint2* ranges, int64_t tiles, const uint32_t* tile_order, uint32_t* point_list,
                           const uint32_t* depth_keys, uint32_t* scratch, hipStream_t s, int debug) {
    if (tiles <= 0) return OGS_OK;
    if (tiles >= (1ll << 31)) { set_error("tile_depth_sort: %lld tiles", (long long)tiles); return OGS_ERR_UNSUPPORTED; }
    const unsigned grid = (unsigned)((tiles + kTileSortWaves - 1) / kTileSortWaves);
    OGS_LAUNCH(tile_depth_sort_kernel, dim3(grid), dim3(kBlock), 0, s, ranges, (int)tiles, tile_order, point_list, depth_keys,
               scratch);
    OGS_LAUNCH_CHECK(debug, s);
    return OGS_OK;
}

int launch_export_keys(const uint2* ranges, int tiles, const uint32_t* point_list, const float4* rec, int recv4,
                       uint64_t* keys_out, hipStream_t s) {
    OGS_LAUNCH(export_keys_kernel, dim3(tiles), dim3(kBlock), 0, s, ranges, point_list, rec, recv4, keys_out);
    OGS_LAUNCH_CHECK(0, s);
    return OGS_OK;
}

}
```

### opengaussian_amd/csrc/capi.hip

```cpp
#include <stdarg.h>
#include <stdlib.h>
#include <string.h>

#include <map>
#include <mutex>
#include <string>
#include <vector>

#include "ogs_common.h"

namespace ogs {

static thread_local char g_err[512] = "";

void set_error(const char* fmt, ...) {
    va_list ap;
    va_start(ap, fmt);
    vsnprintf(g_err, sizeof(g_err), fmt, ap);
    va_end(ap);
}

namespace {
struct ProfRec { const char* name; hipEvent_t start, stop; };
int g_prof_mode = 0;
char g_prof_prefix[64] = "blend_";
std::vector<ProfRec> g_prof;
std::vector<hipEvent_t> g_event_pool;
std::mutex g_prof_mu;
hipEvent_t take_event() {
    if (!g_event_pool.empty()) { hipEvent_t e = g_event_pool.back(); g_event_pool.pop_back(); return e; }
    hipEvent_t e = nullptr;
    (void)hipEventCreate(&e);
    return e;
}
}

ProfScope::ProfScope(const char* n, hipStream_t s) : name(n), stream(s), slot(-1) {
    if (g_prof_mode == 0) return;
    if (g_prof_mode == 2 && strncmp(n, g_prof_prefix, strlen(g_prof_prefix)) != 0) return;
    std::lock_guard<std::mutex> lk(g_prof_mu);
    ProfRec r{n, take_event(), take_event()};
    (void)hipEventRecord(r.start, s);
    g_prof.push_back(r);
    slot = (int)g_prof.size() - 1;
}
ProfScope::~ProfScope() {
    if (slot < 0) return;
    std::lock_guard<std::mutex> lk(g_prof_mu);
    (void)hipEventRecord(g_prof[slot].stop, stream);
}

namespace {
uint32_t* g_async_status = nullptr;
std::mutex g_async_mu;
}
uint32_t* async_status_word() {
    std::lock_guard<std::mutex> lk(g_async_mu);
    if (!g_async_status) {
        void* p = nullptr;
        const hipError_t e = hipHostMalloc(&p, 64, hipHostMallocMapped | hipHostMallocPortable);
        if (e != hipSuccess || !p) {
            set_error("hipHostMalloc of the async status word failed: %s", hipGetErrorString(e));
            return nullptr;
        }
        memset(p, 0, 64);
        g_async_status = static_cast<uint32_t*>(p);
    }
    return g_async_status;
}
int take_async_status() {
    std::lock_guard<std::mutex> lk(g_async_mu);
    if (!g_async_status) return 0;
    return (int)__atomic_exchange_n(g_async_status, 0u, __ATOMIC_ACQ_REL);
}
int check_async_status(const char* where) {
    const int st = take_async_status();
    if (st == 0) return OGS_OK;
    set_error("%s: a kernel of an earlier launch reported status 0x%x%s%s -- the results of the passes since the last check "
              "are not valid", where, st,
              (st & (int)kAsyncRadixSpin) ? " (one-launch radix pass: a look-back wait exceeded its bound)" : "",
              (st & (int)kAsyncSplitOverflow) ? " (query split: the scatter met more rows than its capacity)" : "");
    return OGS_ERR_DEVICE;
}

}
int ogs::blend_prefetch_lines() {
    static const int v = [] {
        const char* e = getenv("OGS_BLEND_PREFETCH");
        const int n = e ? atoi(e) : kPrefetchMax;
        const int lines = (n & 0xFF) > kPrefetchMax ? kPrefetchMax : (n & 0xFF);
#ifdef OGS_EXPERIMENTS
        return n < 0 ? 0 : (lines | (n & 0x300));
#else
        return n < 0 ? 0 : lines;
#endif
    }();
    return v;
}
namespace ogs {

static int bit_length(uint32_t v) {
    int n = 0;
    while (v) { ++n; v >>= 1; }
    return n;
}

static int validate_fwd(const OgsRasterFwdArgs* a, bool images = true) {
    if (!a) { set_error("args == NULL"); return OGS_ERR_INVALID_ARG; }
    if (a->P < 0 || a->W <= 0 || a->H <= 0) { set_error("bad sizes P=%d W=%d H=%d", a->P, a->W, a->H); return OGS_ERR_INVALID_ARG; }
    if (a->C != 3 && a->C != 6 && a->C != 9 && a->C != 12) { set_error("C=%d unsupported (3, 6, 9, 12)", a->C); return OGS_ERR_UNSUPPORTED; }
    if (a->shs == nullptr && a->colors_precomp == nullptr) {
        set_error("provide shs or colors_precomp"); return OGS_ERR_INVALID_ARG;
    }
    if (a->shs != nullptr && (a->colors_precomp != nullptr) != (a->C > 3)) {
        set_error("with shs: C == 3 and no colors_precomp, or C > 3 with colors_precomp holding the C-3 extra channels");
        return OGS_ERR_INVALID_ARG;
    }
    const bool sr = a->scales != nullptr && a->rotations != nullptr;
    if (sr == (a->cov3D_precomp != nullptr) || (a->scales != nullptr) != (a->rotations != nullptr)) {
        set_error("provide exactly one of (scales, rotations) / cov3D_precomp"); return OGS_ERR_INVALID_ARG;
    }
    if (a->shs) {
        if (a->sh_degree < 0 || a->sh_degree > 3 || a->sh_coeffs < (a->sh_degree + 1) * (a->sh_degree + 1)) {
            set_error("sh_degree=%d needs >= %d coefficients, got %d", a->sh_degree, (a->sh_degree + 1) * (a->sh_degree + 1), a->sh_coeffs);
            return OGS_ERR_INVALID_ARG;
        }
    }
    if (!a->bg || !a->viewmatrix || !a->projmatrix || !a->campos || (images && (!a->out_color || !a->out_depth || !a->out_alpha))) {
        set_error("NULL required pointer"); return OGS_ERR_INVALID_ARG;
    }
    if (a->P > 0 && (!a->means3D || !a->opacities || !a->radii || !a->geom_buffer || !a->geom_tmp)) {
        set_error("NULL required per-Gaussian pointer"); return OGS_ERR_INVALID_ARG;
    }
    if (a->num_groups < 0 || (a->num_groups > 1 && a->P > 0 && !a->group_ids)) {
        set_error("num_groups=%d needs group_ids", a->num_groups); return OGS_ERR_INVALID_ARG;
    }
    return OGS_OK;
}

static int validate_raw(const OgsRawModel* raw, int P, int M) {
    if (!raw) { set_error("raw == NULL"); return OGS_ERR_INVALID_ARG; }
    if (M < 1) { set_error("raw model: sh_coeffs=%d < 1", M); return OGS_ERR_INVALID_ARG; }
    if (P > 0 && (!raw->features_dc || !raw->scaling || !raw->rotation || !raw->opacity)) {
        set_error("raw model: NULL features_dc / scaling / rotation / opacity"); return OGS_ERR_INVALID_ARG;
    }
    if (P > 0 && M > 1 && !raw->features_rest) { set_error("raw model: features_rest == NULL with %d SH coefficients", M); return OGS_ERR_INVALID_ARG; }
    return OGS_OK;
}

static int raw_fwd_args(const OgsRasterFwdArgs* a, const OgsRawModel* raw, OgsRasterFwdArgs* out) {
    if (!a) { set_error("args == NULL"); return OGS_ERR_INVALID_ARG; }
    if (a->shs || a->opacities || a->scales || a->rotations || a->cov3D_precomp) {
        set_error("raw pass: args.shs / opacities / scales / rotations / cov3D_precomp must be NULL (the raw model takes their place)");
        return OGS_ERR_INVALID_ARG;
    }
    int rc = validate_raw(raw, a->P, a->sh_coeffs);
    if (rc != OGS_OK) return rc;
    *out = *a;
    out->shs = raw->features_dc;
    out->opacities = raw->opacity;
    out->scales = raw->scaling;
    out->rotations = raw->rotation;
    if (a->P == 0) {
        out->shs = out->scales = out->rotations = a->bg;
    }
    return OGS_OK;
}

}

using namespace ogs;

extern "C" {

int ogs_version(void) { return 408; }

int ogs_check_async_status(void) { return check_async_status("ogs_check_async_status"); }

int ogs_prof_enable(int on) {
    std::lock_guard<std::mutex> lk(g_prof_mu);
    for (auto& r : g_prof) { g_event_pool.push_back(r.start); g_event_pool.push_back(r.stop); }
    g_prof.clear();
    g_prof_mode = on;
    return OGS_OK;
}

int ogs_prof_filter(const char* prefix) {
    std::lock_guard<std::mutex> lk(g_prof_mu);
    if (!prefix || strlen(prefix) >= sizeof(g_prof_prefix)) { set_error("prof_filter: prefix NULL or longer than %zu", sizeof(g_prof_prefix) - 1); return OGS_ERR_INVALID_ARG; }
    strcpy(g_prof_prefix, prefix);
    return OGS_OK;
}

int ogs_prof_collect(char* buf, size_t n) {
    std::lock_guard<std::mutex> lk(g_prof_mu);
    std::map<std::string, std::pair<long, double>> agg;
    for (auto& r : g_prof) {
        OGS_HIP_CHECK(hipEventSynchronize(r.stop));
        float ms = 0.f;
        OGS_HIP_CHECK(hipEventElapsedTime(&ms, r.start, r.stop));
        auto& a = agg[r.name];
        a.first += 1;
        a.second += ms;
    }
    std::string out = "{";
    bool first = true;
    for (auto& kv : agg) {
        char line[384];
        std::string nm = kv.first;
        for (auto& ch : nm) if (ch == '"') ch = '\'';
        snprintf(line, sizeof(line), "%s\"%s\": {\"calls\": %ld, \"total_ms\": %.6f}", first ? "" : ", ", nm.c_str(),
                 kv.second.first, kv.second.second);
        out += line;
        first = false;
    }
    out += "}";
    if (!buf || out.size() + 1 > n) { set_error("prof_collect: buffer too small (%zu needed)", out.size() + 1); return OGS_ERR_SCRATCH_TOO_SMALL; }
    memcpy(buf, out.c_str(), out.size() + 1);
    return OGS_OK;
}
const char* ogs_last_error(void) { return g_err; }

size_t ogs_raster_geom_bytes(int32_t P, int32_t C) { return GeomState::bytes(P > 0 ? P : 1, C); }
size_t ogs_raster_geom_tmp_bytes(int32_t P) { return GeomTmp::bytes(P > 0 ? P : 1); }
size_t ogs_raster_image_bytes(int32_t W, int32_t H) { return ImageState::bytes(W, H); }
size_t ogs_raster_image_bytes_grouped(int32_t W, int32_t H, int32_t G) { return ImageState::bytes(W, H, num_groups_of(G)); }
size_t ogs_raster_binning_tmp_bytes(int64_t D, int32_t, int32_t) { return BinTmp::bytes(D > 0 ? D : 1); }
size_t ogs_raster_sorted_bytes(int64_t D, int32_t C) {
    return align_up((size_t)(D > 0 ? D : 1) * stream_vec4(C) * sizeof(float4));
}
size_t ogs_raster_quad_list_bytes(int64_t D) {
    return align_up((size_t)(5 * (D > 0 ? D : 1) + 2 * kQuadPad) * sizeof(uint32_t));
}
size_t ogs_raster_backward_tmp_bytes(int32_t P) { return align_up((size_t)(P > 0 ? P : 1) * 16 * sizeof(double)); }

static int forward_geometry_impl(const OgsRasterFwdArgs* a_in, void* stream_, int64_t* num_rendered_host, bool raw,
                                 const float* raw_rest) {
    int rc = validate_fwd(a_in, false);
    if (rc != OGS_OK) return rc;
    OgsRasterFwdArgs a_raw;
    const OgsRasterFwdArgs* a = a_in;
    if (raw) { a_raw = *a_in; a_raw.cov3D_precomp = raw_rest; a = &a_raw; }
    hipStream_t s = static_cast<hipStream_t>(stream_);
    if (num_rendered_host) *num_rendered_host = 0;
    if (a->P == 0) return OGS_OK;
    rc = check_async_status("forward (entry)");
    if (rc != OGS_OK) return rc;
    const GeomState gs = GeomState::carve(a->geom_buffer, a->P, a->C);
    const GeomTmp gt = GeomTmp::carve(a->geom_tmp, a->P);
    if (a->P <= kSmallMaxP) {
        rc = launch_small_geometry(*a, gs, gt, s, raw);
        if (rc != OGS_OK) return rc;
    } else if (per_tile_depth_order(*a)) {
        rc = launch_preprocess(*a, gs, gt, s, raw);
        if (rc != OGS_OK) return rc;
        rc = block_sum_offsets(*a) ? launch_block_offsets(*a, gt, s)
                                   : exclusive_scan_u32(gt.tiles_touched, nullptr, gt.offsets, a->P, gt.num_rendered, gt.sort_tmp, s, a->debug);
        if (rc != OGS_OK) return rc;
    } else {
        rc = launch_preprocess(*a, gs, gt, s, raw);
        if (rc != OGS_OK) return rc;
        const bool sweep = radix_onesweep_enabled(a->P);
        if (sweep) {
            const int shifts[4] = {0, 8, 16, 24}, nbits[4] = {8, 8, 8, 8};
            rc = radix_sort_begin(gt.keys[0], a->P, nullptr, 4, shifts, nbits, gt.sort_tmp, s, a->debug, true);
            if (rc != OGS_OK) return rc;
        }
        for (int pass = 0; pass < 4; ++pass) {
            const int in = pass & 1, out = in ^ 1;
            const bool drop = pass == 0;
            const uint32_t* n_pass = drop ? nullptr : gt.visible();
            rc = sweep ? radix_sort_pass(pass, 4, gt.keys[in], gt.order[in], gt.keys[out], gt.order[out], a->P, 8 * pass, 8, gt.sort_tmp, s, a->debug, n_pass, drop, drop ? gt.visible() : nullptr)
                       : radix_pass(gt.keys[in], gt.order[in], gt.keys[out], gt.order[out], a->P, 8 * pass, 8, gt.sort_tmp, s, a->debug, n_pass, drop, drop ? gt.visible() : nullptr);
            if (rc != OGS_OK) return rc;
        }
        rc = exclusive_scan_u32(gt.tiles_touched, gt.order[0], gt.offsets, a->P, gt.num_rendered, gt.sort_tmp, s, a->debug, gt.visible());
        if (rc != OGS_OK) return rc;
    }
    if (num_rendered_host) {
        uint32_t d = 0;
        OGS_HIP_CHECK(hipMemcpyAsync(&d, gt.num_rendered, sizeof(uint32_t), hipMemcpyDeviceToHost, s));
        OGS_HIP_CHECK(hipStreamSynchronize(s));
        *num_rendered_host = (int64_t)d;
        rc = check_async_status("forward geometry phase");
        if (rc != OGS_OK) return rc;
    }
    return OGS_OK;
}

int ogs_raster_forward_geometry(const OgsRasterFwdArgs* a, void* stream_, int64_t* num_rendered_host) {
    return forward_geometry_impl(a, stream_, num_rendered_host, false, nullptr);
}

int ogs_raster_forward_geometry_raw(const OgsRasterFwdArgs* a, const OgsRawModel* raw, void* stream_, int64_t* num_rendered_host) {
    OgsRasterFwdArgs b;
    const int rc = raw_fwd_args(a, raw, &b);
    if (rc != OGS_OK) return rc;
    return forward_geometry_impl(&b, stream_, num_rendered_host, true, raw->features_rest);
}

int ogs_model_activate(int32_t P, int32_t M, const OgsRawModel* raw, float* scales, float* rotations, float* opacities, float* shs,
                       void* stream_) {
    if (P < 0) { set_error("model_activate: P=%d", P); return OGS_ERR_INVALID_ARG; }
    if (P == 0) return OGS_OK;
    if (!raw) { set_error("model_activate: raw == NULL"); return OGS_ERR_INVALID_ARG; }
    if ((scales && !raw->scaling) || (rotations && !raw->rotation) || (opacities && !raw->opacity) ||
        (shs && (M < 1 || !raw->features_dc || (M > 1 && !raw->features_rest)))) {
        set_error("model_activate: an output is requested whose raw input is NULL (M=%d)", M); return OGS_ERR_INVALID_ARG;
    }
    return launch_model_activate(P, M, *raw, scales, rotations, opacities, shs, static_cast<hipStream_t>(stream_));
}

int ogs_raster_read_num_rendered_async(const OgsRasterFwdArgs* a, void* stream_, uint32_t* host_pinned) {
    if (!a || !host_pinned) { set_error("read_num_rendered_async: NULL pointer"); return OGS_ERR_INVALID_ARG; }
    if (a->P == 0) { *host_pinned = 0; return OGS_OK; }
    const GeomTmp gt = GeomTmp::carve(a->geom_tmp, a->P);
    OGS_HIP_CHECK(hipMemcpyAsync(host_pinned, gt.num_rendered, sizeof(uint32_t), hipMemcpyDeviceToHost,
                                 static_cast<hipStream_t>(stream_)));
    return OGS_OK;
}

int ogs_raster_read_num_emitted(const OgsRasterFwdArgs* a, void* stream_, uint32_t* host) {
    if (!a || !host) { set_error("read_num_emitted: NULL pointer"); return OGS_ERR_INVALID_ARG; }
    *host = 0;
    if (a->P == 0) return OGS_OK;
    if (!a->geom_tmp) { set_error("read_num_emitted: geom_tmp == NULL"); return OGS_ERR_INVALID_ARG; }
    const GeomTmp gt = GeomTmp::carve(a->geom_tmp, a->P);
    hipStream_t s = static_cast<hipStream_t>(stream_);
    OGS_HIP_CHECK(hipMemcpyAsync(host, block_sum_offsets(*a) ? gt.emitted() : gt.num_rendered, sizeof(uint32_t), hipMemcpyDeviceToHost, s));
    OGS_HIP_CHECK(hipStreamSynchronize(s));
    return OGS_OK;
}

static int render_impl(const OgsRasterFwdArgs* a, int64_t D, bool deferred, hipStream_t s,
                       const OgsGroupStatsArgs* stats = nullptr) {
    int rc = validate_fwd(a, stats == nullptr);
    if (rc != OGS_OK) return rc;
    if (!a->image_buffer) { set_error("image_buffer == NULL"); return OGS_ERR_INVALID_ARG; }
    if (a->bwd_clear && !stats && (((uintptr_t)a->bwd_clear | a->bwd_clear_bytes) & 15u) != 0) {
        set_error("bwd_clear / bwd_clear_bytes must be multiples of 16"); return OGS_ERR_INVALID_ARG;
    }
    const int G = num_groups_of(a->num_groups);
    const ImageState is = stats ? ImageState::carve_stats(a->image_buffer, a->W, a->H, G)
                                : ImageState::carve(a->image_buffer, a->W, a->H, G);
    const int gx = (a->W + kTile - 1) / kTile, gy = (a->H + kTile - 1) / kTile;
    const int64_t tiles = (int64_t)gx * gy * G;
    if (tiles >= (1ll << 31)) { set_error("%d groups x %d tiles exceed 2^31 virtual tiles", G, gx * gy); return OGS_ERR_UNSUPPORTED; }
    const GeomState gs = GeomState::carve(a->geom_buffer, a->P > 0 ? a->P : 1, a->C);
    const bool per_tile = per_tile_depth_order(*a);
    bool order_ready = false;
    if (D > 0) {
        if (!a->point_list || !a->binning_tmp) { set_error("point_list / binning_tmp == NULL with num_rendered=%lld", (long long)D); return OGS_ERR_INVALID_ARG; }
        if (D >= (1ll << 31)) { set_error("num_rendered=%lld exceeds 2^31", (long long)D); return OGS_ERR_UNSUPPORTED; }
        const GeomTmp gt = GeomTmp::carve(a->geom_tmp, a->P);
        const BinTmp bt = BinTmp::carve(a->binning_tmp, D);
        const int bits = bit_length((uint32_t)(tiles - 1));
        const int passes = bits == 0 ? 1 : (bits + 7) / 8;
        const int per = bits == 0 ? 1 : (bits + passes - 1) / passes;
        uint32_t* vbuf[2];
        vbuf[passes & 1] = a->point_list;
        vbuf[(passes & 1) ^ 1] = bt.vals;
        const uint32_t* n_dev = block_sum_offsets(*a) ? gt.emitted() : deferred ? gt.num_rendered : nullptr;
        const bool cull = a->full_binning == 0;
        const bool zero_in_dup = tiles <= (int64_t)a->P;
        rc = launch_duplicate(*a, gs, gt, bt.tile_keys[0], vbuf[0], (uint32_t)D, cull, !per_tile, s,
                              zero_in_dup ? is.ranges : nullptr, zero_in_dup ? (int)tiles : 0);
        if (rc != OGS_OK) return rc;
        const bool sweep = radix_onesweep_enabled(D);
        int shifts[4], nbits[4];
        for (int p = 0; p < passes; ++p) {
            shifts[p] = p * per;
            nbits[p] = (p == passes - 1) ? (bits == 0 ? 1 : bits - shifts[p]) : per;
        }
        if (passes == 2 && (bits & 1)) {
            nbits[0] = bits / 2; shifts[1] = nbits[0]; nbits[1] = bits - nbits[0];
        }
        if (sweep) {
            rc = radix_sort_begin(bt.tile_keys[0], D, n_dev, passes, shifts, nbits, bt.sort_tmp, s, a->debug, cull);
            if (rc != OGS_OK) return rc;
        }
        for (int p = 0; p < passes; ++p) {
            const int in = p & 1, out = in ^ 1;
            const bool drop = cull && p == 0;
            const uint32_t* n_pass = (cull && p > 0) ? bt.kept : n_dev;
            rc = sweep ? radix_sort_pass(p, passes, bt.tile_keys[in], vbuf[in], bt.tile_keys[out], vbuf[out], D, shifts[p], nbits[p], bt.sort_tmp, s, a->debug, n_pass, drop, drop ? bt.kept : nullptr)
                       : radix_pass(bt.tile_keys[in], vbuf[in], bt.tile_keys[out], vbuf[out], D, shifts[p], nbits[p], bt.sort_tmp, s, a->debug, n_pass, drop, drop ? bt.kept : nullptr);
            if (rc != OGS_OK) return rc;
        }
        rc = launch_tile_ranges(bt.tile_keys[passes & 1], D, is.ranges, tiles, s, a->debug, cull ? bt.kept : n_dev, zero_in_dup);
        if (rc != OGS_OK) return rc;
        if (per_tile) {
            const uint32_t* order = launch_tile_order(is, tiles, a->P, s, a->debug);
            order_ready = true;
            rc = launch_tile_depth_sort(is.ranges, tiles, order, a->point_list, gt.keys[0], bt.vals, s, a->debug);
            if (rc != OGS_OK) return rc;
        }
    } else {
        OGS_HIP_CHECK(hipMemsetAsync(is.ranges, 0, (size_t)tiles * sizeof(uint2), s));
    }
    if (stats) return launch_group_stats(*a, *stats, gs, is, s, order_ready);
    if (!a->sorted_rec || !a->quad_list) { set_error("sorted_rec / quad_list == NULL"); return OGS_ERR_INVALID_ARG; }
    return launch_blend_forward(*a, gs, is, D, s, order_ready);
}

int ogs_raster_forward_render(const OgsRasterFwdArgs* a, int64_t D, void* stream_) {
    return render_impl(a, D, false, static_cast<hipStream_t>(stream_));
}

size_t ogs_raster_stats_image_bytes(int32_t W, int32_t H, int32_t G) {
    return ImageState::stats_bytes(W > 0 ? W : 1, H > 0 ? H : 1, num_groups_of(G));
}
size_t ogs_raster_stats_tmp_bytes(int32_t G, int32_t L, int32_t C) {
    return align_up((size_t)num_groups_of(G) * (size_t)((L > 0 ? L : 0) + 1) * (size_t)(C > 0 ? C : 1) * sizeof(int64_t));
}

int ogs_raster_forward_group_stats(const OgsRasterFwdArgs* a, const OgsGroupStatsArgs* st, int64_t D, void* stream_) {
    if (!a || !st) { set_error("forward_group_stats: NULL argument"); return OGS_ERR_INVALID_ARG; }
    if (st->num_labels < 0) { set_error("forward_group_stats: num_labels=%d < 0", st->num_labels); return OGS_ERR_INVALID_ARG; }
    if (!st->labels || !st->max_alpha || !st->count || !st->feat_sum || !st->stats_tmp) {
        set_error("forward_group_stats: NULL labels / output / stats_tmp pointer"); return OGS_ERR_INVALID_ARG;
    }
    if (D < 0) { set_error("forward_group_stats: num_rendered=%lld < 0", (long long)D); return OGS_ERR_INVALID_ARG; }
    if (a->P == 0) D = 0;
    return render_impl(a, D, false, static_cast<hipStream_t>(stream_), st);
}

int ogs_raster_forward_render_deferred(const OgsRasterFwdArgs* a, int64_t capacity, void* stream_) {
    if (capacity <= 0) { set_error("forward_render_deferred: capacity must be > 0"); return OGS_ERR_INVALID_ARG; }
    return render_impl(a, capacity, true, static_cast<hipStream_t>(stream_));
}

int ogs_raster_forward_reblend(const OgsRasterFwdArgs* a, void* stream_) {
    if (!a) { set_error("args == NULL"); return OGS_ERR_INVALID_ARG; }
    if (a->P <= 0 || a->W <= 0 || a->H <= 0) { set_error("forward_reblend: bad sizes P=%d W=%d H=%d", a->P, a->W, a->H); return OGS_ERR_INVALID_ARG; }
    if (a->C != 3 && a->C != 6 && a->C != 9 && a->C != 12) { set_error("C=%d unsupported (3, 6, 9, 12)", a->C); return OGS_ERR_UNSUPPORTED; }
    if (a->num_groups > 1) { set_error("forward_reblend: grouped passes are not kept"); return OGS_ERR_UNSUPPORTED; }
    if (!a->colors_precomp || !a->bg || !a->out_color || !a->out_depth || !a->out_alpha || !a->image_buffer || !a->sorted_rec ||
        !a->quad_list) {
        set_error("forward_reblend: NULL required pointer (colors_precomp, bg, out_*, image_buffer, sorted_rec, quad_list)");
        return OGS_ERR_INVALID_ARG;
    }
    const int rc = check_async_status("forward_reblend (entry)");
    if (rc != OGS_OK) return rc;
    const ImageState is = ImageState::carve(a->image_buffer, a->W, a->H, 1);
    return launch_reblend(*a, is, static_cast<hipStream_t>(stream_));
}

int ogs_raster_compact_kept(int32_t W, int32_t H, int32_t C, const void* image_buffer, const void* sorted_rec, const void* quad_list,
                            void* new_image_buffer, void* new_sorted_rec, void* new_quad_list, void* stream_) {
    if (W <= 0 || H <= 0) { set_error("compact_kept: bad sizes W=%d H=%d", W, H); return OGS_ERR_INVALID_ARG; }
    if (!image_buffer || !sorted_rec || !quad_list || !new_image_buffer || !new_sorted_rec || !new_quad_list) {
        set_error("compact_kept: NULL pointer"); return OGS_ERR_INVALID_ARG;
    }
    const ImageState is_old = ImageState::carve(const_cast<void*>(image_buffer), W, H, 1);
    const ImageState is_new = ImageState::carve(new_image_buffer, W, H, 1);
    return launch_compact_kept(W, H, C, is_old, is_new, sorted_rec, quad_list, new_sorted_rec, new_quad_list,
                               static_cast<hipStream_t>(stream_));
}

size_t ogs_raster_tiny_max_points(void) { return (size_t)kTinyMaxP; }

size_t ogs_raster_tile_sort_capacity(int32_t level) {
    return level == 0 ? (size_t)kWaveSortCap : level == 1 ? (size_t)kTileSortCap : 0;
}

static int forward_tiny_impl(const OgsRasterFwdArgs* a_in, void* stream_, bool raw, const float* raw_rest) {
    int rc = validate_fwd(a_in);
    if (rc != OGS_OK) return rc;
    OgsRasterFwdArgs a_raw;
    const OgsRasterFwdArgs* a = a_in;
    if (raw) { a_raw = *a_in; a_raw.cov3D_precomp = raw_rest; a = &a_raw; }
    if (a->P <= 0 || a->P > kTinyMaxP) { set_error("forward_tiny: P=%d outside [1, %d]", a->P, kTinyMaxP); return OGS_ERR_INVALID_ARG; }
    if (a->num_groups > 1) { set_error("forward_tiny: grouped passes use the streaming path"); return OGS_ERR_UNSUPPORTED; }
    hipStream_t s = static_cast<hipStream_t>(stream_);
    const GeomState gs = GeomState::carve(a->geom_buffer, a->P, a->C);
    uint32_t* order = static_cast<uint32_t*>(a->geom_tmp);
    rc = launch_tiny_geometry(*a, gs, order, s, raw);
    if (rc != OGS_OK) return rc;
    return launch_tiny_blend(*a, gs, order, s);
}

int ogs_raster_forward_tiny(const OgsRasterFwdArgs* a, void* stream_) { return forward_tiny_impl(a, stream_, false, nullptr); }

int ogs_raster_forward_tiny_raw(const OgsRasterFwdArgs* a, const OgsRawModel* raw, void* stream_) {
    OgsRasterFwdArgs b;
    const int rc = raw_fwd_args(a, raw, &b);
    if (rc != OGS_OK) return rc;
    return forward_tiny_impl(&b, stream_, true, raw->features_rest);
}

static int backward_impl(const OgsRasterBwdArgs* a, void* stream_, const OgsRawModelGrads* raw_grads) {
    if (!a) { set_error("args == NULL"); return OGS_ERR_INVALID_ARG; }
    if (a->C != 3 && a->C != 6 && a->C != 9) { set_error("backward: C=%d unsupported (3, 6, 9)", a->C); return OGS_ERR_UNSUPPORTED; }
    if (a->P == 0) return OGS_OK;
    const bool feat_only = backward_is_features_only(*a);
    if (!a->dL_dcolor || !a->image_buffer || !a->bwd_tmp || !a->radii) {
        set_error("backward: NULL required pointer"); return OGS_ERR_INVALID_ARG;
    }
    if (!feat_only && (!a->geom_buffer || !a->bg || !a->means3D || !a->viewmatrix || !a->projmatrix || !a->campos)) {
        set_error("backward: NULL required pointer"); return OGS_ERR_INVALID_ARG;
    }
    if (!feat_only && a->num_rendered > 0 && !a->point_list) { set_error("backward: point_list == NULL"); return OGS_ERR_INVALID_ARG; }
    if ((int64_t)a->P * grad_stride(a->C) >= (1ll << 32)) {
        set_error("backward: P=%d exceeds the %lld Gaussians the 32-bit gradient-record offsets address", a->P,
                  (long long)((1ll << 32) / grad_stride(a->C)) - 1);
        return OGS_ERR_UNSUPPORTED;
    }
    {
        const int st = check_async_status("backward (entry)");
        if (st != OGS_OK) return st;
    }
    hipStream_t s = static_cast<hipStream_t>(stream_);
    const GeomState gs = GeomState::carve(const_cast<void*>(a->geom_buffer), a->P, a->C);
    if (a->num_groups < 0) { set_error("backward: num_groups=%d", a->num_groups); return OGS_ERR_INVALID_ARG; }
    const ImageState is = ImageState::carve(const_cast<void*>(a->image_buffer), a->W, a->H, num_groups_of(a->num_groups));
    void* grad_rec = a->bwd_tmp;
    const int rec_doubles = feat_only ? feat_grad_stride(a->C, a->shs ? 3 : 0) : grad_stride(a->C);
    if (!a->bwd_tmp_is_clear) OGS_HIP_CHECK(hipMemsetAsync(grad_rec, 0, (size_t)a->P * rec_doubles * sizeof(double), s));
    if (a->num_rendered > 0 && (!a->sorted_rec || !a->quad_list)) { set_error("backward: sorted_rec / quad_list == NULL"); return OGS_ERR_INVALID_ARG; }
    int rc = launch_blend_backward(*a, is, grad_rec, s);
    if (rc != OGS_OK) return rc;
    return launch_preprocess_backward(*a, gs, grad_rec, s, raw_grads);
}

int ogs_raster_backward(const OgsRasterBwdArgs* a, void* stream_) { return backward_impl(a, stream_, nullptr); }

int ogs_raster_backward_raw(const OgsRasterBwdArgs* a, const OgsRawModel* raw, const OgsRawModelGrads* grads, void* stream_) {
    if (!a) { set_error("args == NULL"); return OGS_ERR_INVALID_ARG; }
    if (a->shs || a->opacities || a->scales || a->rotations || a->cov3D_precomp || a->dL_dsh || a->dL_dopacity || a->dL_dscales ||
        a->dL_drotations || a->dL_dcov3D) {
        set_error("raw backward: args.shs / opacities / scales / rotations / cov3D_precomp and their dL_d* outputs must be NULL "
                  "(the raw model and its gradient struct take their place)");
        return OGS_ERR_INVALID_ARG;
    }
    const int rc = validate_raw(raw, a->P, a->sh_coeffs);
    if (rc != OGS_OK) return rc;
    static const OgsRawModelGrads kNoGrads = {nullptr, nullptr, nullptr, nullptr, nullptr};
    const OgsRawModelGrads* g = grads ? grads : &kNoGrads;
    if (g->features_rest && !raw->features_rest) { set_error("raw backward: a features_rest gradient without features_rest"); return OGS_ERR_INVALID_ARG; }
    OgsRasterBwdArgs b = *a;
    b.shs = raw->features_dc;
    b.opacities = raw->opacity;
    b.scales = raw->scaling;
    b.rotations = raw->rotation;
    b.cov3D_precomp = raw->features_rest;
    b.dL_dsh = g->features_dc ? g->features_dc : g->features_rest;
    b.dL_dopacity = g->opacity;
    b.dL_dscales = g->scaling;
    b.dL_drotations = g->rotation;
    return backward_impl(&b, stream_, g);
}

int ogs_mark_visible(int32_t P, const float* means3D, const float* viewmatrix, const float*, uint8_t* present,
                     void* stream_) {
    if (P == 0) return OGS_OK;
    if (!means3D || !viewmatrix || !present) { set_error("mark_visible: NULL pointer"); return OGS_ERR_INVALID_ARG; }
    return launch_mark_visible(P, means3D, viewmatrix, present, static_cast<hipStream_t>(stream_));
}

int ogs_sh_grad_from_views(int32_t P, int32_t V, int32_t sh_degree, int32_t sh_coeffs, const float* means3D,
                           const float* campos, const float* dL_drgb, float* dL_dsh, void* stream_) {
    if (P == 0) return OGS_OK;
    if (P < 0 || V < 1 || sh_degree < 0 || sh_degree > 3 || sh_coeffs < (sh_degree + 1) * (sh_degree + 1)) {
        set_error("sh_grad_from_views: bad sizes P=%d V=%d degree=%d coeffs=%d", P, V, sh_degree, sh_coeffs);
        return OGS_ERR_INVALID_ARG;
    }
    if (!means3D || !campos || !dL_drgb || !dL_dsh) { set_error("sh_grad_from_views: NULL pointer"); return OGS_ERR_INVALID_ARG; }
    return launch_sh_grad_from_views(P, V, sh_degree, sh_coeffs, means3D, campos, dL_drgb, dL_dsh,
                                     static_cast<hipStream_t>(stream_));
}

int ogs_selftest_wave_fold16(const float* in, float* out, void* stream_) {
    if (!in || !out) { set_error("selftest: NULL pointer"); return OGS_ERR_INVALID_ARG; }
    return launch_wave_fold16_test(in, out, static_cast<hipStream_t>(stream_));
}

int ogs_selftest_mfma_rank1(const float* w, const float* f, const float* acc0, int32_t steps, float* out_mfma, float* out_fma,
                            void* stream_) {
    if (!w || !f || !acc0 || !out_mfma || !out_fma || steps < 0) { set_error("selftest: NULL pointer / steps < 0"); return OGS_ERR_INVALID_ARG; }
    return launch_mfma_rank1_test(w, f, acc0, steps, out_mfma, out_fma, static_cast<hipStream_t>(stream_));
}

int ogs_selftest_tile_order(const uint32_t* ranges, int64_t vtiles, uint32_t* order, void* stream_) {
    if (!ranges || !order || vtiles <= 0) { set_error("selftest: NULL pointer / no tiles"); return OGS_ERR_INVALID_ARG; }
    return launch_tile_order_test(ranges, vtiles, order, static_cast<hipStream_t>(stream_));
}

size_t ogs_selftest_radix_tmp_bytes(int64_t n) { return sort_tmp_bytes(n > 0 ? n : 1); }

int ogs_selftest_radix_sort(uint32_t* keys0, uint32_t* vals0, uint32_t* keys1, uint32_t* vals1, int64_t n, int32_t key_bits,
                            int32_t variant, int32_t items, const uint32_t* n_dev, void* tmp, int32_t* result_buffer,
                            void* stream_) {
    if (!result_buffer) { set_error("selftest_radix_sort: NULL result_buffer"); return OGS_ERR_INVALID_ARG; }
    *result_buffer = 0;
    if (n <= 0) return OGS_OK;
    if (items != 0 && items != 4 && items != 16) { set_error("selftest_radix_sort: items=%d (0, 4 or 16)", items); return OGS_ERR_INVALID_ARG; }
    if (!keys0 || !vals0 || !keys1 || !vals1 || !tmp || key_bits < 1 || key_bits > 32) {
        set_error("selftest_radix_sort: bad arguments"); return OGS_ERR_INVALID_ARG;
    }
    hipStream_t s = static_cast<hipStream_t>(stream_);
    uint32_t* k[2] = {keys0, keys1};
    uint32_t* v[2] = {vals0, vals1};
    const int passes = (key_bits + 7) / 8, per = (key_bits + passes - 1) / passes;
    int shifts[4], nbits[4];
    for (int p = 0; p < passes; ++p) { shifts[p] = p * per; nbits[p] = p == passes - 1 ? key_bits - shifts[p] : per; }
    const bool sweep = (variant & 1) != 0, drop = (variant & 2) != 0;
    const int spin_limit = (variant & 4) ? 0 : -1;
    (void)take_async_status();
    uint32_t* kept = nullptr;
    if (drop) {
        OGS_HIP_CHECK(hipMalloc(&kept, sizeof(uint32_t)));
        OGS_HIP_CHECK(hipMemsetAsync(kept, 0xA5, sizeof(uint32_t), s));
    }
    int rc = OGS_OK;
    if (sweep) rc = radix_sort_begin(k[0], n, n_dev, passes, shifts, nbits, tmp, s, 0, drop, items);
    for (int p = 0; p < passes && rc == OGS_OK; ++p) {
        const int in = p & 1, out = in ^ 1;
        const bool d0 = drop && p == 0;
        const uint32_t* n_pass = (drop && p > 0) ? kept : n_dev;
        rc = sweep ? radix_sort_pass(p, passes, k[in], v[in], k[out], v[out], n, shifts[p], nbits[p], tmp, s, 0, n_pass, d0, d0 ? kept : nullptr, items, spin_limit)
                   : radix_pass(k[in], v[in], k[out], v[out], n, shifts[p], nbits[p], tmp, s, 0, n_pass, d0, d0 ? kept : nullptr);
    }
    uint32_t kept_host = 0;
    if (drop) {
        if (rc == OGS_OK && hipMemcpyAsync(&kept_host, kept, sizeof(uint32_t), hipMemcpyDeviceToHost, s) != hipSuccess) rc = OGS_ERR_HIP;
        (void)hipStreamSynchronize(s);
        (void)hipFree(kept);
    } else {
        (void)hipStreamSynchronize(s);
    }
    if (rc != OGS_OK) return rc;
    *result_buffer = (passes & 1) | (drop ? (int32_t)(kept_host << 1) : 0);
    return check_async_status("selftest_radix_sort");
}

int ogs_raster_export_binning(const OgsRasterFwdArgs* a, int64_t D, uint64_t* keys_out, uint32_t* ranges_out,
                              uint32_t* n_contrib_out, void* stream_) {
    if (!a) { set_error("args == NULL"); return OGS_ERR_INVALID_ARG; }
    hipStream_t s = static_cast<hipStream_t>(stream_);
    const int G = num_groups_of(a->num_groups);
    const ImageState is = ImageState::carve(a->image_buffer, a->W, a->H, G);
    const int gx = (a->W + kTile - 1) / kTile, gy = (a->H + kTile - 1) / kTile;
    if (keys_out && D > 0) {
        const GeomState gs = GeomState::carve(a->geom_buffer, a->P, a->C);
        int rc = launch_export_keys(is.ranges, gx * gy * G, a->point_list, gs.rec, rec_vec4(a->C), keys_out, s);
        if (rc != OGS_OK) return rc;
    }
    if (ranges_out)
        OGS_HIP_CHECK(hipMemcpyAsync(ranges_out, is.ranges, (size_t)gx * gy * G * sizeof(uint2), hipMemcpyDeviceToDevice, s));
    if (n_contrib_out) {
        if (D > 0) {
            int rc = launch_export_n_contrib(*a, is, n_contrib_out, s);
            if (rc != OGS_OK) return rc;
        } else {
            OGS_HIP_CHECK(hipMemsetAsync(n_contrib_out, 0, (size_t)G * a->W * a->H * sizeof(uint32_t), s));
        }
    }
    return OGS_OK;
}

}
```

### opengaussian_amd/csrc/ogs_common.h

```cpp
#pragma once

#include <hip/hip_runtime.h>
#include <stdint.h>
#include <stddef.h>
#include <stdio.h>
#include <type_traits>

#include "../../include/ogs_raster.h"
#include "../../include/ogs_model.h"

namespace ogs {

constexpr int kTile = OGS_TILE;
constexpr int kBlock = 256;
constexpr int kWave = 64;
constexpr int kTinyMaxP = 256;
constexpr int kSmallMaxP = 1024;

void set_error(const char* fmt, ...);

#define OGS_HIP_CHECK(expr)                                                              \
    do {                                                                                 \
        hipError_t _e = (expr);                                                          \
        if (_e != hipSuccess) {                                                          \
            ogs::set_error("%s failed: %s (%s:%d)", #expr, hipGetErrorString(_e), __FILE__, __LINE__); \
            return OGS_ERR_HIP;                                                          \
        }                                                                                \
    } while (0)

#define OGS_LAUNCH_CHECK(debug, stream)                                                  \
    do {                                                                                 \
        OGS_HIP_CHECK(hipGetLastError());                                                \
        if (debug) OGS_HIP_CHECK(hipStreamSynchronize(stream));                          \
    } while (0)

constexpr uint32_t kAsyncRadixSpin = 1u;
constexpr uint32_t kAsyncSplitOverflow = 2u;
uint32_t* async_status_word();
int take_async_status();
int check_async_status(const char* where);

struct ProfScope {
    const char* name;
    hipStream_t stream;
    int slot;
    ProfScope(const char* name, hipStream_t s);
    ~ProfScope();
};
#define OGS_LAUNCH(kernel, grid, block, lds, stream, ...)                      \
    do {                                                                       \
        ogs::ProfScope _ps(#kernel, stream);                                   \
        hipLaunchKernelGGL(kernel, grid, block, lds, stream, __VA_ARGS__);     \
    } while (0)

#define OGS_LAUNCH_NAMED(name, kernel, grid, block, lds, stream, ...)          \
    do {                                                                       \
        ogs::ProfScope _ps(name, stream);                                      \
        hipLaunchKernelGGL(kernel, grid, block, lds, stream, __VA_ARGS__);     \
    } while (0)
template <int C>
constexpr const char* chan_name(const char* const (&names)[4]) {
    return C == 3 ? names[0] : C == 6 ? names[1] : C == 9 ? names[2] : names[3];
}

template <int MaxC, class F>
int dispatch_channels(int C, const char* unsupported_fmt, F&& f) {
    static_assert(MaxC == 9 || MaxC == 12, "supported sets: {3, 6, 9} and {3, 6, 9, 12}");
    switch (C) {
        case 3: return f(std::integral_constant<int, 3>{});
        case 6: return f(std::integral_constant<int, 6>{});
        case 9: return f(std::integral_constant<int, 9>{});
        case 12:
            if constexpr (MaxC >= 12) return f(std::integral_constant<int, 12>{});
            [[fallthrough]];
        default: set_error(unsupported_fmt, C); return OGS_ERR_UNSUPPORTED;
    }
}

constexpr size_t kAlign = 256;
inline size_t align_up(size_t v, size_t a = kAlign) { return (v + a - 1) / a * a; }

struct Carver {
    char* base;
    size_t off = 0;
    explicit Carver(void* p) : base(static_cast<char*>(p)) {}
    template <typename T>
    T* take(size_t n) {
        T* r = reinterpret_cast<T*>(base ? base + off : nullptr);
        off = align_up(off + n * sizeof(T));
        return r;
    }
};

__host__ __device__ constexpr int rec_vec4(int C) { return 2 + (C + 3) / 4; }

__host__ __device__ constexpr int stream_vec4(int C) { return (8 + C + 1 + 3) / 4; }

constexpr int kQuadPad = 16;
template <int C>
inline float4* stream_base(void* buf) { return static_cast<float4*>(buf); }
inline uint32_t* quad_base(void* buf) { return static_cast<uint32_t*>(buf) + kQuadPad; }
constexpr float kFar = 3.0e18f;
constexpr float kFarTest = 1.0e18f;

typedef float f8 __attribute__((ext_vector_type(8)));
template <int C>
struct StreamRec {
    static constexpr int NF4 = stream_vec4(C) - 2;
    f8 g;
    float4 f[NF4];
    __device__ __forceinline__ void load(const float* __restrict__ p) {
        g = *reinterpret_cast<const f8*>(p);
#pragma unroll
        for (int k = 0; k < NF4; ++k) f[k] = *reinterpret_cast<const float4*>(p + 8 + 4 * k);
    }
    __device__ __forceinline__ float feat(int c) const {
        const float4 v = f[c >> 2];
        return (c & 3) == 0 ? v.x : (c & 3) == 1 ? v.y : (c & 3) == 2 ? v.z : v.w;
    }
};

constexpr int kSlotDepth = 9, kSlotMoments = 10;
__host__ __device__ constexpr int grad_stride(int C) { return (C + 7 <= 16) ? 16 : 32; }
__host__ __device__ constexpr int feat_grad_stride(int C, int F0) { return (C - F0 <= 8) ? 8 : grad_stride(C); }

struct GeomState {
    float4* rec;
    uint32_t* clamped;
    static GeomState carve(void* p, int P, int C) {
        Carver c(p);
        GeomState g;
        g.rec = c.take<float4>((size_t)P * rec_vec4(C));
        g.clamped = c.take<uint32_t>(P);
        return g;
    }
    static size_t bytes(int P, int C) {
        Carver c(nullptr);
        c.take<float4>((size_t)P * rec_vec4(C));
        c.take<uint32_t>(P);
        return c.off;
    }
};

struct ImageState {
    uint2* ranges;
    uint32_t* n_contrib;
    uint32_t* qcount;
    float* final_T;
    uint32_t* tile_order;
    static ImageState carve(void* p, int W, int H, int G = 1) {
        Carver c(p);
        ImageState s;
        const size_t tiles = (size_t)G * ((W + kTile - 1) / kTile) * ((H + kTile - 1) / kTile);
        s.ranges = c.take<uint2>(tiles);
        s.n_contrib = c.take<uint32_t>((size_t)G * W * H);
        s.qcount = c.take<uint32_t>(tiles * 5);
        s.final_T = c.take<float>((size_t)G * W * H);
        s.tile_order = c.take<uint32_t>(tiles);
        return s;
    }
    static size_t bytes(int W, int H, int G = 1) {
        Carver c(nullptr);
        const size_t tiles = (size_t)G * ((W + kTile - 1) / kTile) * ((H + kTile - 1) / kTile);
        c.take<uint2>(tiles);
        c.take<uint32_t>((size_t)G * W * H);
        c.take<uint32_t>(tiles * 5);
        c.take<float>((size_t)G * W * H);
        c.take<uint32_t>(tiles);
        return c.off;
    }
    static ImageState carve_stats(void* p, int W, int H, int G) {
        Carver c(p);
        ImageState s{};
        const size_t tiles = (size_t)G * ((W + kTile - 1) / kTile) * ((H + kTile - 1) / kTile);
        s.ranges = c.take<uint2>(tiles);
        s.tile_order = c.take<uint32_t>(tiles);
        return s;
    }
    static size_t stats_bytes(int W, int H, int G) {
        Carver c(nullptr);
        const size_t tiles = (size_t)G * ((W + kTile - 1) / kTile) * ((H + kTile - 1) / kTile);
        c.take<uint2>(tiles);
        c.take<uint32_t>(tiles);
        return c.off;
    }
};
const uint32_t* launch_tile_order(const ImageState& is, int64_t vtiles, int P, hipStream_t s, int debug);
const uint32_t* tile_order_of(const ImageState& is, int64_t vtiles, int P);
int launch_export_n_contrib(const OgsRasterFwdArgs& a, const ImageState& is, uint32_t* out, hipStream_t s);

constexpr int kSortItemsLarge = 8;
inline int sort_items_for(int64_t n) { return n <= (int64_t)(3 << 20) ? 4 : kSortItemsLarge; }
inline int sort_blocks_for(int64_t n) {
    const int64_t tile = (int64_t)kBlock * sort_items_for(n);
    return (int)((n + tile - 1) / tile);
}
size_t scan_tmp_bytes(int64_t n);
size_t sort_tmp_bytes(int64_t n);

int exclusive_scan_u32(const uint32_t* in, const uint32_t* gather, uint32_t* out, int64_t n,
                       uint32_t* total, void* tmp, hipStream_t stream, int debug, const uint32_t* n_dev = nullptr);
constexpr uint32_t kDropKey = 0xFFFFFFFFu;
bool radix_onesweep_enabled(int64_t n);
int radix_sort_begin(const uint32_t* keys, int64_t n, const uint32_t* n_dev, int npass, const int* shifts, const int* bits,
                     void* tmp, hipStream_t stream, int debug, bool drop = false, int items = 0);
int radix_sort_pass(int pass, int npass, const uint32_t* keys_in, const uint32_t* vals_in, uint32_t* keys_out,
                    uint32_t* vals_out, int64_t n, int shift, int bits, void* tmp, hipStream_t stream, int debug,
                    const uint32_t* n_dev = nullptr, bool drop = false, uint32_t* kept_out = nullptr, int items = 0,
                    int spin_limit = -1);
int radix_pass(const uint32_t* keys_in, const uint32_t* vals_in, uint32_t* keys_out, uint32_t* vals_out,
               int64_t n, int shift, int bits, void* tmp, hipStream_t stream, int debug,
               const uint32_t* n_dev = nullptr, bool drop = false, uint32_t* kept_out = nullptr);

constexpr int kBlockSumPad = 8;
__host__ __device__ constexpr int block_sum_run(int nb) { return (nb + kBlockSumPad - 1) / kBlockSumPad * kBlockSumPad; }

struct GeomTmp {
    uint32_t* tiles_touched;
    uint32_t* keys[2];
    uint32_t* order[2];
    uint32_t* offsets;
    uint32_t* num_rendered;
    void* sort_tmp;
    uint32_t* block_sum;
    uint2* emit_rect;
    static constexpr int kEmittedWord = 2;
    uint32_t* visible() const { return num_rendered + 1; }
    uint32_t* emitted() const { return num_rendered + kEmittedWord; }
    static GeomTmp carve(void* p, int P) {
        Carver c(p);
        GeomTmp g;
        g.tiles_touched = c.take<uint32_t>(P);
        g.keys[0] = c.take<uint32_t>(P);
        g.keys[1] = c.take<uint32_t>(P);
        g.order[0] = c.take<uint32_t>(P);
        g.order[1] = c.take<uint32_t>(P);
        g.offsets = c.take<uint32_t>(P);
        g.num_rendered = c.take<uint32_t>(64);
        g.sort_tmp = c.take<char>(sort_tmp_bytes(P));
        g.block_sum = c.take<uint32_t>(2 * (size_t)block_sum_run((P + kBlock - 1) / kBlock));
        g.emit_rect = c.take<uint2>(P);
        return g;
    }
    static size_t bytes(int P) {
        Carver c(nullptr);
        for (int i = 0; i < 6; ++i) c.take<uint32_t>(P);
        c.take<uint32_t>(64);
        c.take<char>(sort_tmp_bytes(P));
        c.take<uint32_t>(2 * (size_t)block_sum_run((P + kBlock - 1) / kBlock));
        c.take<uint2>(P);
        return c.off;
    }
};

struct BinTmp {
    uint32_t* tile_keys[2];
    uint32_t* vals;
    uint32_t* kept;
    void* sort_tmp;
    static BinTmp carve(void* p, int64_t D) {
        Carver c(p);
        BinTmp b;
        b.tile_keys[0] = c.take<uint32_t>(D);
        b.tile_keys[1] = c.take<uint32_t>(D);
        b.vals = c.take<uint32_t>(D);
        b.kept = c.take<uint32_t>(1);
        b.sort_tmp = c.take<char>(sort_tmp_bytes(D));
        return b;
    }
    static size_t bytes(int64_t D) {
        Carver c(nullptr);
        for (int i = 0; i < 3; ++i) c.take<uint32_t>(D);
        c.take<uint32_t>(1);
        c.take<char>(sort_tmp_bytes(D));
        return c.off;
    }
};

int launch_preprocess(const OgsRasterFwdArgs& a, const GeomState& gs, const GeomTmp& gt, hipStream_t s, bool raw = false);
int launch_block_offsets(const OgsRasterFwdArgs& a, const GeomTmp& gt, hipStream_t s);
int launch_tiny_geometry(const OgsRasterFwdArgs& a, const GeomState& gs, uint32_t* order, hipStream_t s, bool raw = false);
int launch_small_geometry(const OgsRasterFwdArgs& a, const GeomState& gs, const GeomTmp& gt, hipStream_t s, bool raw = false);
int launch_model_activate(int P, int M, const OgsRawModel& raw, float* scales, float* rotations, float* opacities, float* shs,
                          hipStream_t s);
int launch_tiny_blend(const OgsRasterFwdArgs& a, const GeomState& gs, const uint32_t* order, hipStream_t s);
int launch_reblend(const OgsRasterFwdArgs& a, const ImageState& is, hipStream_t s);
int launch_compact_kept(int W, int H, int C, const ImageState& is_old, const ImageState& is_new, const void* old_rec,
                        const void* old_quad, void* new_rec, void* new_quad, hipStream_t s);
int launch_duplicate(const OgsRasterFwdArgs& a, const GeomState& gs, const GeomTmp& gt, uint32_t* tile_keys,
                     uint32_t* vals, uint32_t capacity, bool drop_unreachable, bool depth_order, hipStream_t s,
                     uint2* zero_ranges = nullptr, int n_zero = 0);
int launch_tile_ranges(const uint32_t* tile_keys_sorted, int64_t D, uint2* ranges, int64_t tiles, hipStream_t s,
                       int debug, const uint32_t* n_dev = nullptr, bool already_zeroed = false);
inline bool per_tile_depth_order(const OgsRasterFwdArgs& a) { return a.num_groups <= 1 && a.P > kSmallMaxP; }
inline bool block_sum_offsets(const OgsRasterFwdArgs& a) { return per_tile_depth_order(a) && a.full_binning == 0; }
constexpr int kTileSortItems = 16;
constexpr int kTileSortCap = kBlock * kTileSortItems;
constexpr int kWaveSortCap = kTileSortCap / (kBlock / kWave);
int launch_tile_depth_sort(const uint2* ranges, int64_t tiles, const uint32_t* tile_order, uint32_t* point_list,
                           const uint32_t* depth_keys, uint32_t* scratch, hipStream_t s, int debug);
inline int num_groups_of(int g) { return g > 1 ? g : 1; }
int launch_group_stats(const OgsRasterFwdArgs& a, const OgsGroupStatsArgs& st, const GeomState& gs, const ImageState& is,
                       hipStream_t s, bool order_ready = false);
int launch_blend_forward(const OgsRasterFwdArgs& a, const GeomState& gs, const ImageState& is, int64_t D,
                         hipStream_t s, bool order_ready = false);
int launch_blend_backward(const OgsRasterBwdArgs& a, const ImageState& is, void* grad_rec, hipStream_t s);
int launch_preprocess_backward(const OgsRasterBwdArgs& a, const GeomState& gs, const void* grad_rec, hipStream_t s,
                               const OgsRawModelGrads* raw_grads = nullptr);
inline bool backward_is_features_only(const OgsRasterBwdArgs& a) {
    return a.dL_dcolors != nullptr && a.colors_precomp != nullptr && !a.dL_dmeans2D && !a.dL_dopacity &&
           !a.dL_dmeans3D && !a.dL_dcov3D && !a.dL_dsh && !a.dL_dscales && !a.dL_drotations && !a.dL_dsh_rgb;
}
int launch_sh_grad_from_views(int P, int V, int sh_degree, int sh_coeffs, const float* means3D, const float* campos,
                              const float* dL_drgb, float* dL_dsh, hipStream_t s);
int launch_wave_fold16_test(const float* in, float* out, hipStream_t s);
int launch_mfma_rank1_test(const float* w, const float* f, const float* acc0, int steps, float* out_mfma, float* out_fma,
                           hipStream_t s);
int launch_tile_order_test(const uint32_t* ranges, int64_t vtiles, uint32_t* order, hipStream_t s);
int launch_mark_visible(int P, const float* means3D, const float* viewmatrix, uint8_t* present, hipStream_t s);
int launch_export_keys(const uint2* ranges, int tiles, const uint32_t* point_list, const float4* rec, int recv4,
                       uint64_t* keys_out, hipStream_t s);

__device__ __forceinline__ float blend_power(float a2, float b2, float c2, float dx, float dy) {
    const float u = fmaf(b2, dy, a2 * dx);
    return fmaf(c2 * dy, dy, u * dx);
}

constexpr int kPrefetchMax = 4;
struct RecordPrefetch {
    uint32_t v[kPrefetchMax];
    __device__ __forceinline__ void issue(const float* __restrict__ tile_records, int n_tile, int rec_floats, int tid,
                                          int lines) {
        const uint32_t total = (uint32_t)n_tile * (uint32_t)rec_floats;
#pragma unroll
        for (int k = 0; k < kPrefetchMax; ++k) {
            v[k] = 0u;
            const uint32_t off = ((uint32_t)(k * kBlock + tid)) * 32u;
            if (k < lines && off < total) v[k] = __float_as_uint(tile_records[off]);
        }
    }
    __device__ __forceinline__ void retire(uint32_t* __restrict__ sink, int never) const {
        const uint32_t x = v[0] ^ v[1] ^ v[2] ^ v[3];
        if (never < 0 && x == 0x7FC12345u) sink[0] = x;
    }
};
int blend_prefetch_lines();

constexpr float kThrMargin = 0.01f;
constexpr int kReachBit = 31;
constexpr uint32_t kGidMask = (1u << kReachBit) - 1u;
__device__ __forceinline__ float max_power_in_box(float A, float B, float Cc, float nbA, float nbC, float xlo, float xhi,
                                                  float ylo, float yhi) {
    if (xlo <= 0.f && xhi >= 0.f && ylo <= 0.f && yhi >= 0.f) return 0.f;
    auto q = [&](float dx, float dy) { return -0.5f * (A * dx * dx + Cc * dy * dy) - B * dx * dy; };
    float m = q(xlo, fminf(fmaxf(nbC * xlo, ylo), yhi));
    m = fmaxf(m, q(xhi, fminf(fmaxf(nbC * xhi, ylo), yhi)));
    m = fmaxf(m, q(fminf(fmaxf(nbA * ylo, xlo), xhi), ylo));
    m = fmaxf(m, q(fminf(fmaxf(nbA * yhi, xlo), xhi), yhi));
    const float X = fmaxf(fabsf(xlo), fabsf(xhi)), Y = fmaxf(fabsf(ylo), fabsf(yhi));
    return m + 8e-7f * (0.5f * (A * X * X + Cc * Y * Y) + fabsf(B) * X * Y);
}
__device__ __forceinline__ float max_power_in_box(float A, float B, float Cc, float xlo, float xhi, float ylo,
                                                  float yhi) {
    return max_power_in_box(A, B, Cc, -B / A, -B / Cc, xlo, xhi, ylo, yhi);
}

__device__ __forceinline__ void wait_scalar_loads() {
    __builtin_amdgcn_sched_barrier(0);
    __builtin_amdgcn_s_waitcnt(0xC07F);
    __builtin_amdgcn_sched_barrier(0);
}
__device__ __forceinline__ int lane_id() { return threadIdx.x & (kWave - 1); }
__device__ __forceinline__ void lds_barrier() { asm volatile("s_waitcnt lgkmcnt(0)\n\ts_barrier" ::: "memory"); }

}
```

Before: 1513 Mpix/s.

## Replace tile-key radix sort with counting-sort binning and id-stable tile sorts

When per-tile depth ordering applies, tile binning now uses a three-kernel counting sort (per-block LDS histograms, a column scan over the per-block count table, then an atomic placement pass) instead of multi-pass radix sorting followed by a tile-range search. It also produces the tile ranges and the kept count directly. Because atomic placement does not keep input order, the per-tile wave and block depth sorts now detect equal-depth ties that are out of gaussian-id order and re-sort by id to restore determinism. The aim is to cut the global radix passes, at the cost of LDS atomic contention and possible extra sort passes inside tiles.

```diff
diff --git a/include/ogs_raster.h b/include/ogs_raster.h
--- a/include/ogs_raster.h
+++ b/include/ogs_raster.h
@@ -126,6 +126,9 @@
 
 size_t ogs_raster_tile_sort_capacity(int32_t level);
 
+int ogs_raster_tile_count_debug(int64_t D, int64_t tiles, int32_t force_blocks, int32_t reverse);
+size_t ogs_raster_tile_count_trip(void);
+
 int ogs_raster_forward_reblend(const OgsRasterFwdArgs* args, void* stream);
 
 int ogs_raster_compact_kept(int32_t W, int32_t H, int32_t C, const void* image_buffer, const void* sorted_rec,
diff --git a/opengaussian_amd/_lib.py b/opengaussian_amd/_lib.py
--- a/opengaussian_amd/_lib.py
+++ b/opengaussian_amd/_lib.py
@@ -113,6 +113,8 @@
     "ogs_raster_backward": (C.c_int, [C.POINTER(OgsRasterBwdArgs), _vp]),
     "ogs_raster_tiny_max_points": (C.c_size_t, []),
     "ogs_raster_tile_sort_capacity": (C.c_size_t, [C.c_int32]),
+    "ogs_raster_tile_count_debug": (C.c_int, [C.c_int64, C.c_int64, C.c_int32, C.c_int32]),
+    "ogs_raster_tile_count_trip": (C.c_size_t, []),
     "ogs_raster_forward_tiny": (C.c_int, [C.POINTER(OgsRasterFwdArgs), _vp]),
     "ogs_raster_forward_reblend": (C.c_int, [C.POINTER(OgsRasterFwdArgs), _vp]),
     "ogs_raster_compact_kept": (C.c_int, [C.c_int32, C.c_int32, C.c_int32, _vp, _vp, _vp, _vp, _vp, _vp, _vp]),
diff --git a/opengaussian_amd/csrc/binning.hip b/opengaussian_amd/csrc/binning.hip
--- a/opengaussian_amd/csrc/binning.hip
+++ b/opengaussian_amd/csrc/binning.hip
@@ -455,6 +455,147 @@
     }
 }
 
+constexpr int kCountBlock = 1024;
+constexpr int kCountItems = 4;
+constexpr int kCountTrip = kCountBlock * kCountItems;
+constexpr int kCountScanCols = 64, kCountScanGroups = 16;
+
+__device__ __forceinline__ void tile_count_chunk(const uint32_t* __restrict__ n_dev, int64_t n_cap, int nchunks, int64_t& begin,
+                                                 int64_t& end) {
+    const int64_t n = n_dev ? min((int64_t)*n_dev, n_cap) : n_cap;
+    const int64_t per = (n + nchunks - 1) / nchunks;
+    const int64_t chunk = (per + kCountTrip - 1) / kCountTrip * kCountTrip;
+    begin = min(n, (int64_t)blockIdx.x * chunk);
+    end = min(n, begin + chunk);
+}
+
+__global__ __launch_bounds__(kCountBlock) void tile_count_kernel(const uint32_t* __restrict__ keys, int64_t n_cap,
+                                                                 const uint32_t* __restrict__ n_dev, int tiles,
+                                                                 uint32_t* __restrict__ table ) {
+    extern __shared__ uint32_t count_lds[];
+    int64_t begin, end;
+    tile_count_chunk(n_dev, n_cap, (int)gridDim.x, begin, end);
+    for (int t = threadIdx.x; t < tiles; t += kCountBlock) count_lds[t] = 0u;
+    __syncthreads();
+    for (int64_t i0 = begin + (int64_t)threadIdx.x * kCountItems; i0 < end; i0 += kCountTrip) {
+        uint32_t k[kCountItems];
+        if (i0 + kCountItems <= end) {
+            const uint4 v = *reinterpret_cast<const uint4*>(keys + i0);
+            k[0] = v.x; k[1] = v.y; k[2] = v.z; k[3] = v.w;
+        } else {
+#pragma unroll
+            for (int j = 0; j < kCountItems; ++j) k[j] = i0 + j < end ? keys[i0 + j] : kDropKey;
+        }
+#pragma unroll
+        for (int j = 0; j < kCountItems; ++j)
+            if (k[j] < (uint32_t)tiles) atomicAdd(&count_lds[k[j]], 1u);
+    }
+    __syncthreads();
+    uint32_t* row = table + (size_t)blockIdx.x * tiles;
+    for (int t = threadIdx.x; t < tiles; t += kCountBlock) row[t] = count_lds[t];
+}
+
+__global__ __launch_bounds__(kCountScanCols * kCountScanGroups) void tile_count_scan_kernel(uint32_t* __restrict__ table, int nrows,
+                                                                                            int tiles) {
+    __shared__ uint32_t part[kCountScanGroups][kCountScanCols];
+    const int c = threadIdx.x & (kCountScanCols - 1), g = threadIdx.x / kCountScanCols;
+    const int t = blockIdx.x * kCountScanCols + c;
+    const int per = (nrows + kCountScanGroups - 1) / kCountScanGroups;
+    const int r0 = min(nrows, g * per), r1 = min(nrows, r0 + per);
+    uint32_t sum = 0;
+    if (t < tiles) {
+#pragma unroll 8
+        for (int r = r0; r < r1; ++r) sum += table[(size_t)r * tiles + t];
+    }
+    part[g][c] = sum;
+    __syncthreads();
+    uint32_t run = 0, total = 0;
+#pragma unroll
+    for (int j = 0; j < kCountScanGroups; ++j) {
+        const uint32_t v = part[j][c];
+        if (j < g) run += v;
+        total += v;
+    }
+    if (t >= tiles) return;
+    if (g == 0) table[(size_t)nrows * tiles + t] = total;
+#pragma unroll 8
+    for (int r = r0; r < r1; ++r) {
+        uint32_t* p = table + (size_t)r * tiles + t;
+        const uint32_t v = *p;
+        *p = run;
+        run += v;
+    }
+}
+
+__global__ __launch_bounds__(kCountBlock) void tile_place_kernel(const uint32_t* __restrict__ keys, const uint32_t* __restrict__ vals,
+                                                                 int64_t n_cap, const uint32_t* __restrict__ n_dev, int tiles,
+                                                                 const uint32_t* __restrict__ table, uint2* __restrict__ ranges,
+                                                                 uint32_t* __restrict__ kept, uint32_t* __restrict__ out,
+                                                                 uint32_t out_cap, bool reverse) {
+    extern __shared__ uint32_t count_lds[];
+    __shared__ uint32_t wave_sums[kCountBlock / kWave];
+    int64_t begin, end;
+    tile_count_chunk(n_dev, n_cap, (int)gridDim.x, begin, end);
+    if (begin >= end && blockIdx.x != 0) return;
+    const uint32_t* totals = table + (size_t)gridDim.x * tiles;
+    const uint32_t* row = table + (size_t)blockIdx.x * tiles;
+    for (int t = threadIdx.x; t < tiles; t += kCountBlock) count_lds[t] = totals[t];
+    __syncthreads();
+    const int per = ((tiles + kCountBlock - 1) / kCountBlock) | 1;
+    const int t0 = min(tiles, (int)threadIdx.x * per), t1 = min(tiles, t0 + per);
+    uint32_t sum = 0;
+    for (int t = t0; t < t1; ++t) sum += count_lds[t];
+    const uint32_t inc = wave_inclusive_scan(sum);
+    if (lane_id() == kWave - 1) wave_sums[threadIdx.x >> 6] = inc;
+    __syncthreads();
+    uint32_t run = inc - sum, total = 0;
+#pragma unroll
+    for (int w = 0; w < kCountBlock / kWave; ++w) {
+        const uint32_t v = wave_sums[w];
+        if (w < (int)(threadIdx.x >> 6)) run += v;
+        total += v;
+    }
+    for (int t = t0; t < t1; ++t) {
+        const uint32_t cnt = count_lds[t];
+        count_lds[t] = run;
+        run += cnt;
+    }
+    __syncthreads();
+    if (blockIdx.x == 0) {
+        for (int t = threadIdx.x; t < tiles; t += kCountBlock) {
+            const uint32_t cnt = totals[t], start = count_lds[t];
+            ranges[t] = cnt ? make_uint2(start, start + cnt) : make_uint2(0u, 0u);
+        }
+        if (threadIdx.x == 0) *kept = total;
+    }
+    for (int t = threadIdx.x; t < tiles; t += kCountBlock) count_lds[t] += row[t];
+    __syncthreads();
+    for (int64_t j0 = (int64_t)threadIdx.x * kCountItems; j0 < end - begin; j0 += kCountTrip) {
+        uint32_t k[kCountItems], v[kCountItems];
+        if (!reverse && begin + j0 + kCountItems <= end) {
+            const uint4 kk = *reinterpret_cast<const uint4*>(keys + begin + j0);
+            const uint4 vv = *reinterpret_cast<const uint4*>(vals + begin + j0);
+            k[0] = kk.x; k[1] = kk.y; k[2] = kk.z; k[3] = kk.w;
+            v[0] = vv.x; v[1] = vv.y; v[2] = vv.z; v[3] = vv.w;
+        } else {
+#pragma unroll
+            for (int j = 0; j < kCountItems; ++j) {
+                const int64_t i = reverse ? end - 1 - (j0 + j) : begin + j0 + j;
+                const bool in = j0 + j < end - begin;
+                k[j] = in ? keys[i] : kDropKey;
+                v[j] = in ? vals[i] : 0u;
+            }
+        }
+#pragma unroll
+        for (int j = 0; j < kCountItems; ++j) {
+            if (k[j] < (uint32_t)tiles) {
+                const uint32_t pos = atomicAdd(&count_lds[k[j]], 1u);
+                if (pos < out_cap) out[pos] = v[j];
+            }
+        }
+    }
+}
+
 constexpr int kTileSortWaves = kBlock / kWave;
 struct TileSortLds {
     uint32_t hist[kTileSortWaves][256];
@@ -507,6 +648,7 @@
     }
 }
 
+template <bool BY_ID = false>
 __device__ __forceinline__ void load_items(const uint32_t* __restrict__ list, const uint32_t* __restrict__ depth_keys,
                                            uint32_t (&key)[kTileSortItems], uint32_t (&val)[kTileSortItems], int ipl, int first,
                                            int m) {
@@ -518,8 +660,28 @@
 #pragma unroll
     for (int i = 0; i < kTileSortItems; ++i) {
         if (i >= ipl) continue;
-        key[i] = depth_keys[val[i] & kGidMask];
-    }
+        key[i] = BY_ID ? val[i] & kGidMask : depth_keys[val[i] & kGidMask];
+    }
+}
+
+__device__ __forceinline__ void wave_and_or(const uint32_t (&w)[kTileSortItems], int ipl, uint32_t keep, uint32_t& k_and,
+                                            uint32_t& k_or) {
+    k_and = 0xFFFFFFFFu; k_or = 0u;
+#pragma unroll
+    for (int i = 0; i < kTileSortItems; ++i) {
+        if (i >= ipl) continue;
+        k_and &= w[i] & keep;
+        k_or |= w[i] & keep;
+    }
+#pragma unroll
+    for (int d = 32; d >= 1; d >>= 1) {
+        k_and &= (uint32_t)__shfl_xor((int)k_and, d, kWave);
+        k_or |= (uint32_t)__shfl_xor((int)k_or, d, kWave);
+    }
+}
+
+__device__ __forceinline__ bool tie_out_of_order(uint32_t k0, uint32_t v0, uint32_t k1, uint32_t v1) {
+    return k0 == k1 && (v0 & kGidMask) > (v1 & kGidMask);
 }
 
 __device__ __forceinline__ uint32_t tile_sort_rank(TileSortLds& sm, const uint32_t (&key)[kTileSortItems],
@@ -542,6 +704,53 @@
     sm.dig_start[tid] = block_exclusive_scan(run_len, total, sm.scan_sums);
     __syncthreads();
     return run_len;
+}
+
+__device__ __forceinline__ void wave_lsd_passes(LdsWord* hist, LdsMask* masks, LdsWord* wk, LdsWord* wv,
+                                                const uint32_t (&sel)[kTileSortItems], uint32_t (&key)[kTileSortItems],
+                                                uint32_t (&val)[kTileSortItems], uint32_t (&rank)[kTileSortItems], int ipl,
+                                                int n, uint32_t diff, bool reload_last) {
+    const int lane = threadIdx.x & (kWave - 1);
+    const int lo = __builtin_ctz(diff), hi = 31 - __builtin_clz(diff);
+    const int npass = (hi - lo + 8) / 8;
+    const int per = (hi - lo + npass) / npass;
+    for (int p = 0; p < npass; ++p) {
+        const int shift = lo + p * per, bits = min(per, hi + 1 - shift);
+        const uint32_t mask = (1u << bits) - 1u;
+        wave_rank_clear(hist, masks);
+        wave_rank(hist, masks, sel, rank, ipl, 0, n, shift, mask);
+        uint32_t c[4], sum = 0;
+#pragma unroll
+        for (int j = 0; j < 4; ++j) { c[j] = hist[4 * lane + j]; sum += c[j]; }
+        uint32_t run = wave_inclusive_scan(sum) - sum;
+#pragma unroll
+        for (int j = 0; j < 4; ++j) { hist[4 * lane + j] = run; run += c[j]; }
+        __builtin_amdgcn_wave_barrier();
+#pragma unroll
+        for (int i = 0; i < kTileSortItems; ++i) {
+            if (i >= ipl) continue;
+            rank[i] += hist[(sel[i] >> shift) & mask];
+        }
+#pragma unroll
+        for (int i = 0; i < kTileSortItems; ++i) {
+            if (i >= ipl) continue;
+            if (i * kWave + lane < n) {
+                wk[rank[i]] = key[i];
+                wv[rank[i]] = val[i];
+            }
+        }
+        __builtin_amdgcn_wave_barrier();
+        if (p + 1 < npass || reload_last) {
+#pragma unroll
+            for (int i = 0; i < kTileSortItems; ++i) {
+                if (i >= ipl) continue;
+                const int e = min(i * kWave + lane, n - 1);
+                key[i] = wk[e];
+                val[i] = wv[e];
+            }
+            __builtin_amdgcn_wave_barrier();
+        }
+    }
 }
 
 __device__ __forceinline__ void wave_sort_list(TileSortLds& sm, uint32_t* __restrict__ seg, int n,
@@ -554,138 +763,111 @@
     uint32_t key[kTileSortItems], val[kTileSortItems], rank[kTileSortItems];
     const int ipl = (n + kWave - 1) / kWave;
     load_items(seg, depth_keys, key, val, ipl, lane, n);
-    uint32_t k_and = 0xFFFFFFFFu, k_or = 0u;
+    uint32_t k_and, k_or;
+    wave_and_or(key, ipl, 0xFFFFFFFFu, k_and, k_or);
+    const uint32_t kdiff = (uint32_t)__builtin_amdgcn_readfirstlane((int)(k_and ^ k_or));
+    if (kdiff != 0u) {
+        wave_lsd_passes(hist, masks, wk, wv, key, key, val, rank, ipl, n, kdiff, false);
+    } else {
+#pragma unroll
+        for (int i = 0; i < kTileSortItems; ++i) {
+            if (i >= ipl) continue;
+            if (i * kWave + lane < n) { wk[i * kWave + lane] = key[i]; wv[i * kWave + lane] = val[i]; }
+        }
+        __builtin_amdgcn_wave_barrier();
+    }
+    bool bad = false;
 #pragma unroll
     for (int i = 0; i < kTileSortItems; ++i) {
         if (i >= ipl) continue;
-        k_and &= key[i];
-        k_or |= key[i];
-    }
+        const int e = min(i * kWave + lane, n - 2);
+        if (wk[e] == wk[e + 1]) bad |= (wv[e] & kGidMask) > (wv[e + 1] & kGidMask);
+    }
+    if (__ballot(bad) != 0ull) {
+#pragma unroll
+        for (int i = 0; i < kTileSortItems; ++i) {
+            if (i >= ipl) continue;
+            const int e = min(i * kWave + lane, n - 1);
+            key[i] = wk[e];
+            val[i] = wv[e];
+        }
+        __builtin_amdgcn_wave_barrier();
+        wave_and_or(val, ipl, kGidMask, k_and, k_or);
+        const uint32_t gdiff = (uint32_t)__builtin_amdgcn_readfirstlane((int)(k_and ^ k_or));
+        if (gdiff != 0u) wave_lsd_passes(hist, masks, wk, wv, val, key, val, rank, ipl, n, gdiff, kdiff != 0u);
+        if (kdiff != 0u) wave_lsd_passes(hist, masks, wk, wv, key, key, val, rank, ipl, n, kdiff, false);
+    } else if (kdiff == 0u) {
+        return;
+    }
+    for (int j = lane; j < n; j += kWave) seg[j] = wv[j];
+}
+
+__device__ __forceinline__ uint32_t block_and_or(TileSortLds& sm, uint32_t k_and, uint32_t k_or, uint32_t& all_or) {
+    const int tid = threadIdx.x;
 #pragma unroll
     for (int d = 32; d >= 1; d >>= 1) {
         k_and &= (uint32_t)__shfl_xor((int)k_and, d, kWave);
         k_or |= (uint32_t)__shfl_xor((int)k_or, d, kWave);
     }
-    const uint32_t diff = (uint32_t)__builtin_amdgcn_readfirstlane((int)(k_and ^ k_or));
-    if (diff == 0u) return;
-    const int lo = __builtin_ctz(diff), hi = 31 - __builtin_clz(diff);
-    const int npass = (hi - lo + 8) / 8;
-    const int per = (hi - lo + npass) / npass;
-    for (int p = 0; p < npass; ++p) {
-        const int shift = lo + p * per, bits = min(per, hi + 1 - shift);
-        const uint32_t mask = (1u << bits) - 1u;
-        wave_rank_clear(hist, masks);
-        wave_rank(hist, masks, key, rank, ipl, 0, n, shift, mask);
-        uint32_t c[4], sum = 0;
-#pragma unroll
-        for (int j = 0; j < 4; ++j) { c[j] = hist[4 * lane + j]; sum += c[j]; }
-        uint32_t run = wave_inclusive_scan(sum) - sum;
-#pragma unroll
-        for (int j = 0; j < 4; ++j) { hist[4 * lane + j] = run; run += c[j]; }
-        __builtin_amdgcn_wave_barrier();
-#pragma unroll
-        for (int i = 0; i < kTileSortItems; ++i) {
-            if (i >= ipl) continue;
-            rank[i] += hist[(key[i] >> shift) & mask];
-        }
-#pragma unroll
-        for (int i = 0; i < kTileSortItems; ++i) {
-            if (i >= ipl) continue;
-            if (i * kWave + lane < n) {
-                wk[rank[i]] = key[i];
-                wv[rank[i]] = val[i];
-            }
-        }
-        __builtin_amdgcn_wave_barrier();
-        if (p + 1 < npass) {
-#pragma unroll
-            for (int i = 0; i < kTileSortItems; ++i) {
-                if (i >= ipl) continue;
-                const int e = min(i * kWave + lane, n - 1);
-                key[i] = wk[e];
-                val[i] = wv[e];
-            }
-            __builtin_amdgcn_wave_barrier();
-        }
-    }
-    for (int j = lane; j < n; j += kWave) seg[j] = wv[j];
-}
-
-__device__ __forceinline__ void block_sort_list(TileSortLds& sm, uint32_t* __restrict__ seg, uint32_t* __restrict__ alt, int n,
-                                                const uint32_t* __restrict__ depth_keys) {
+    __syncthreads();
+    if (tid < 2) sm.red[tid] = tid == 0 ? 0xFFFFFFFFu : 0u;
+    __syncthreads();
+    if ((tid & (kWave - 1)) == 0) { atomicAnd(&sm.red[0], k_and); atomicOr(&sm.red[1], k_or); }
+    __syncthreads();
+    all_or = sm.red[1];
+    return sm.red[0] ^ all_or;
+}
+
+__device__ __forceinline__ void block_lsd_passes(TileSortLds& sm, const uint32_t (&sel)[kTileSortItems],
+                                                 uint32_t (&key)[kTileSortItems], uint32_t (&val)[kTileSortItems],
+                                                 uint32_t (&rank)[kTileSortItems], int ipl, int chunk, int n, uint32_t diff,
+                                                 bool reload_last) {
     const int tid = threadIdx.x, lane = tid & 63, wave = tid >> 6;
-    const bool in_lds = n <= kTileSortCap;
-    uint32_t key[kTileSortItems], val[kTileSortItems], rank[kTileSortItems];
-    __syncthreads();
-    if (tid < 2) sm.red[tid] = tid == 0 ? 0xFFFFFFFFu : 0u;
-    uint32_t k_and = 0xFFFFFFFFu, k_or = 0u;
-    const int ipl0 = (min(n, kTileSortCap) + kBlock - 1) / kBlock, chunk0 = ipl0 * kWave;
-    if (in_lds) {
-        load_items(seg, depth_keys, key, val, ipl0, wave * chunk0 + lane, n);
-#pragma unroll
-        for (int i = 0; i < kTileSortItems; ++i) {
-            if (i >= ipl0) continue;
-            k_and &= key[i];
-            k_or |= key[i];
-        }
-    } else {
-        for (int j = tid; j < n; j += kBlock) {
-            const uint32_t k = depth_keys[seg[j] & kGidMask];
-            k_and &= k;
-            k_or |= k;
-        }
-    }
-#pragma unroll
-    for (int d = 32; d >= 1; d >>= 1) {
-        k_and &= (uint32_t)__shfl_xor((int)k_and, d, kWave);
-        k_or |= (uint32_t)__shfl_xor((int)k_or, d, kWave);
-    }
-    __syncthreads();
-    if (lane == 0) { atomicAnd(&sm.red[0], k_and); atomicOr(&sm.red[1], k_or); }
-    __syncthreads();
-    const uint32_t diff = sm.red[0] ^ sm.red[1];
-    if (diff == 0u) return;
     const int lo = __builtin_ctz(diff), hi = 31 - __builtin_clz(diff);
     const int npass = (hi - lo + 8) / 8;
     const int per = (hi - lo + npass) / npass;
     uint32_t* const sk = sm.kv;
     uint32_t* const sv = sm.kv + kTileSortCap;
-
-    if (in_lds) {
-        for (int p = 0; p < npass; ++p) {
-            const int shift = lo + p * per, bits = min(per, hi + 1 - shift);
-            const uint32_t mask = (1u << bits) - 1u;
-            tile_sort_rank(sm, key, rank, ipl0, chunk0, n, shift, mask);
+    for (int p = 0; p < npass; ++p) {
+        const int shift = lo + p * per, bits = min(per, hi + 1 - shift);
+        const uint32_t mask = (1u << bits) - 1u;
+        tile_sort_rank(sm, sel, rank, ipl, chunk, n, shift, mask);
+#pragma unroll
+        for (int i = 0; i < kTileSortItems; ++i) {
+            if (i >= ipl) continue;
+            const uint32_t d = (sel[i] >> shift) & mask;
+            rank[i] += sm.dig_start[d] + sm.hist[wave][d];
+        }
+#pragma unroll
+        for (int i = 0; i < kTileSortItems; ++i) {
+            if (i >= ipl) continue;
+            if (wave * chunk + i * kWave + lane < n) {
+                sk[rank[i]] = key[i];
+                sv[rank[i]] = val[i];
+            }
+        }
+        __syncthreads();
+        if (p + 1 < npass || reload_last) {
 #pragma unroll
             for (int i = 0; i < kTileSortItems; ++i) {
-                if (i >= ipl0) continue;
-                const uint32_t d = (key[i] >> shift) & mask;
-                rank[i] += sm.dig_start[d] + sm.hist[wave][d];
-            }
-#pragma unroll
-            for (int i = 0; i < kTileSortItems; ++i) {
-                if (i >= ipl0) continue;
-                if (wave * chunk0 + i * kWave + lane < n) {
-                    sk[rank[i]] = key[i];
-                    sv[rank[i]] = val[i];
-                }
+                if (i >= ipl) continue;
+                const int e = min(wave * chunk + i * kWave + lane, n - 1);
+                key[i] = sk[e];
+                val[i] = sv[e];
             }
             __syncthreads();
-            if (p + 1 < npass) {
-#pragma unroll
-                for (int i = 0; i < kTileSortItems; ++i) {
-                    if (i >= ipl0) continue;
-                    const int e = min(wave * chunk0 + i * kWave + lane, n - 1);
-                    key[i] = sk[e];
-                    val[i] = sv[e];
-                }
-                __syncthreads();
-            }
-        }
-        for (int j = tid; j < n; j += kBlock) seg[j] = sv[j];
-        return;
-    }
-
+        }
+    }
+}
+
+template <bool BY_ID>
+__device__ __forceinline__ void long_lsd_passes(TileSortLds& sm, uint32_t* __restrict__ seg, uint32_t* __restrict__ alt, int n,
+                                                const uint32_t* __restrict__ depth_keys, uint32_t diff) {
+    const int tid = threadIdx.x, lane = tid & 63, wave = tid >> 6;
+    uint32_t key[kTileSortItems], val[kTileSortItems], rank[kTileSortItems];
+    const int lo = __builtin_ctz(diff), hi = 31 - __builtin_clz(diff);
+    const int npass = (hi - lo + 8) / 8;
+    const int per = (hi - lo + npass) / npass;
     for (int p = 0; p < npass; ++p) {
         const int shift = lo + p * per, bits = min(per, hi + 1 - shift);
         const uint32_t mask = (1u << bits) - 1u;
@@ -693,7 +875,10 @@
         uint32_t* __restrict__ dst = (p & 1) ? seg : alt;
         sm.base[tid] = 0u;
         __syncthreads();
-        for (int j = tid; j < n; j += kBlock) atomicAdd(&sm.base[(depth_keys[src[j] & kGidMask] >> shift) & mask], 1u);
+        for (int j = tid; j < n; j += kBlock) {
+            const uint32_t v = src[j] & kGidMask;
+            atomicAdd(&sm.base[((BY_ID ? v : depth_keys[v]) >> shift) & mask], 1u);
+        }
         __syncthreads();
         uint32_t total;
         const uint32_t start = block_exclusive_scan(sm.base[tid], total, sm.scan_sums);
@@ -701,7 +886,7 @@
         for (int c0 = 0; c0 < n; c0 += kTileSortCap) {
             const int m = min(kTileSortCap, n - c0);
             const int ipl = (m + kBlock - 1) / kBlock, chunk = ipl * kWave;
-            load_items(src + c0, depth_keys, key, val, ipl, wave * chunk + lane, m);
+            load_items<BY_ID>(src + c0, depth_keys, key, val, ipl, wave * chunk + lane, m);
             const uint32_t cnt = tile_sort_rank(sm, key, rank, ipl, chunk, m, shift, mask);
 #pragma unroll
             for (int i = 0; i < kTileSortItems; ++i) {
@@ -718,8 +903,91 @@
     }
     if (npass & 1) {
         for (int j = tid; j < n; j += kBlock) seg[j] = alt[j];
-    }
-}
+        __syncthreads();
+    }
+}
+
+__device__ __forceinline__ void block_sort_list(TileSortLds& sm, uint32_t* __restrict__ seg, uint32_t* __restrict__ alt, int n,
+                                                const uint32_t* __restrict__ depth_keys) {
+    const int tid = threadIdx.x, lane = tid & 63, wave = tid >> 6;
+    uint32_t any;
+    __syncthreads();
+    if (n <= kTileSortCap) {
+        uint32_t key[kTileSortItems], val[kTileSortItems], rank[kTileSortItems];
+        uint32_t* const sk = sm.kv;
+        uint32_t* const sv = sm.kv + kTileSortCap;
+        const int ipl = (n + kBlock - 1) / kBlock, chunk = ipl * kWave;
+        load_items(seg, depth_keys, key, val, ipl, wave * chunk + lane, n);
+        uint32_t k_and = 0xFFFFFFFFu, k_or = 0u;
+#pragma unroll
+        for (int i = 0; i < kTileSortItems; ++i) {
+            if (i >= ipl) continue;
+            k_and &= key[i];
+            k_or |= key[i];
+        }
+        const uint32_t kdiff = block_and_or(sm, k_and, k_or, any);
+        if (kdiff != 0u) {
+            block_lsd_passes(sm, key, key, val, rank, ipl, chunk, n, kdiff, false);
+        } else {
+#pragma unroll
+            for (int i = 0; i < kTileSortItems; ++i) {
+                if (i >= ipl) continue;
+                const int e = wave * chunk + i * kWave + lane;
+                if (e < n) { sk[e] = key[i]; sv[e] = val[i]; }
+            }
+            __syncthreads();
+        }
+        bool bad = false;
+#pragma unroll
+        for (int i = 0; i < kTileSortItems; ++i) {
+            if (i >= ipl) continue;
+            const int e = min(wave * chunk + i * kWave + lane, n - 2);
+            if (sk[e] == sk[e + 1]) bad |= (sv[e] & kGidMask) > (sv[e + 1] & kGidMask);
+        }
+        block_and_or(sm, 0xFFFFFFFFu, bad ? 1u : 0u, any);
+        if (any != 0u) {
+            k_and = 0xFFFFFFFFu; k_or = 0u;
+#pragma unroll
+            for (int i = 0; i < kTileSortItems; ++i) {
+                if (i >= ipl) continue;
+                const int e = min(wave * chunk + i * kWave + lane, n - 1);
+                key[i] = sk[e];
+                val[i] = sv[e];
+                k_and &= val[i] & kGidMask;
+                k_or |= val[i] & kGidMask;
+            }
+            const uint32_t gdiff = block_and_or(sm, k_and, k_or, any);
+            if (gdiff != 0u) block_lsd_passes(sm, val, key, val, rank, ipl, chunk, n, gdiff, kdiff != 0u);
+            if (kdiff != 0u) block_lsd_passes(sm, key, key, val, rank, ipl, chunk, n, kdiff, false);
+        } else if (kdiff == 0u) {
+            return;
+        }
+        for (int j = tid; j < n; j += kBlock) seg[j] = sv[j];
+        return;
+    }
+
+    uint32_t k_and = 0xFFFFFFFFu, k_or = 0u;
+    for (int j = tid; j < n; j += kBlock) {
+        const uint32_t k = depth_keys[seg[j] & kGidMask];
+        k_and &= k;
+        k_or |= k;
+    }
+    const uint32_t kdiff = block_and_or(sm, k_and, k_or, any);
+    if (kdiff != 0u) long_lsd_passes<false>(sm, seg, alt, n, depth_keys, kdiff);
+    bool bad = false;
+    k_and = 0xFFFFFFFFu; k_or = 0u;
+    for (int j = tid; j < n; j += kBlock) {
+        const uint32_t v0 = seg[j], v1 = seg[min(j + 1, n - 1)];
+        bad |= tie_out_of_order(depth_keys[v0 & kGidMask], v0, depth_keys[v1 & kGidMask], v1);
+        k_and &= v0 & kGidMask;
+        k_or |= v0 & kGidMask;
+    }
+    const uint32_t gdiff = block_and_or(sm, k_and, k_or | (bad ? 0x80000000u : 0u), any) & kGidMask;
+    if ((any & 0x80000000u) == 0u || gdiff == 0u) return;
+    long_lsd_passes<true>(sm, seg, alt, n, depth_keys, gdiff);
+    if (kdiff != 0u) long_lsd_passes<false>(sm, seg, alt, n, depth_keys, kdiff);
+}
+
 
 __global__ __launch_bounds__(kBlock) void tile_depth_sort_kernel(const uint2* __restrict__ ranges, int tiles,
                                                                  const uint32_t* __restrict__ tile_order,
@@ -933,6 +1201,39 @@
     return OGS_OK;
 }
 
+static int g_tile_count_force = 0;
+static bool g_tile_place_reverse = false;
+void tile_count_debug(int force_blocks, int reverse) {
+    if (force_blocks >= 0) g_tile_count_force = force_blocks;
+    if (reverse >= 0) g_tile_place_reverse = reverse != 0;
+}
+int tile_count_trip() { return kCountTrip; }
+
+int tile_count_blocks(int64_t D, int64_t tiles) {
+    if (tiles < 1 || tiles > kTileCountMaxTiles || D < 2 * tiles) return 0;
+    const int64_t trips = (D + kCountTrip - 1) / kCountTrip;
+    int64_t B = g_tile_count_force > 0 ? g_tile_count_force : (trips < kTileCountBlocks ? trips : kTileCountBlocks);
+    if (B > D / tiles - 1) B = D / tiles - 1;
+    return (int)B;
+}
+
+int launch_tile_count_binning(const uint32_t* keys, const uint32_t* vals, int64_t D, const uint32_t* n_dev, int B, int64_t tiles,
+                              uint32_t* table, uint2* ranges, uint32_t* kept, uint32_t* point_list, hipStream_t s, int debug) {
+    if (B < 1 || tiles < 1 || tiles > kTileCountMaxTiles || ((int64_t)B + 1) * tiles > D) {
+        set_error("tile_count_binning: B=%d tiles=%lld D=%lld", B, (long long)tiles, (long long)D); return OGS_ERR_INVALID_ARG;
+    }
+    const size_t lds = (size_t)tiles * sizeof(uint32_t);
+    OGS_LAUNCH(tile_count_kernel, dim3(B), dim3(kCountBlock), lds, s, keys, D, n_dev, (int)tiles, table);
+    OGS_LAUNCH_CHECK(debug, s);
+    const int cols = (int)((tiles + kCountScanCols - 1) / kCountScanCols);
+    OGS_LAUNCH(tile_count_scan_kernel, dim3(cols), dim3(kCountScanCols * kCountScanGroups), 0, s, table, B, (int)tiles);
+    OGS_LAUNCH_CHECK(debug, s);
+    OGS_LAUNCH(tile_place_kernel, dim3(B), dim3(kCountBlock), lds, s, keys, vals, D, n_dev, (int)tiles, (const uint32_t*)table,
+               ranges, kept, point_list, (uint32_t)D, g_tile_place_reverse);
+    OGS_LAUNCH_CHECK(debug, s);
+    return OGS_OK;
+}
+
 int launch_tile_depth_sort(const uint2* ranges, int64_t tiles, const uint32_t* tile_order, uint32_t* point_list,
                            const uint32_t* depth_keys, uint32_t* scratch, hipStream_t s, int debug) {
     if (tiles <= 0) return OGS_OK;
diff --git a/opengaussian_amd/csrc/capi.hip b/opengaussian_amd/csrc/capi.hip
--- a/opengaussian_amd/csrc/capi.hip
+++ b/opengaussian_amd/csrc/capi.hip
@@ -173,7 +173,7 @@
 
 extern "C" {
 
-int ogs_version(void) { return 408; }
+int ogs_version(void) { return 409; }
 
 int ogs_check_async_status(void) { return check_async_status("ogs_check_async_status"); }
 
@@ -362,33 +362,42 @@
         vbuf[(passes & 1) ^ 1] = bt.vals;
         const uint32_t* n_dev = block_sum_offsets(*a) ? gt.emitted() : deferred ? gt.num_rendered : nullptr;
         const bool cull = a->full_binning == 0;
-        const bool zero_in_dup = tiles <= (int64_t)a->P;
-        rc = launch_duplicate(*a, gs, gt, bt.tile_keys[0], vbuf[0], (uint32_t)D, cull, !per_tile, s,
-                              zero_in_dup ? is.ranges : nullptr, zero_in_dup ? (int)tiles : 0);
-        if (rc != OGS_OK) return rc;
-        const bool sweep = radix_onesweep_enabled(D);
-        int shifts[4], nbits[4];
-        for (int p = 0; p < passes; ++p) {
-            shifts[p] = p * per;
-            nbits[p] = (p == passes - 1) ? (bits == 0 ? 1 : bits - shifts[p]) : per;
+        const int count_blocks = block_sum_offsets(*a) ? tile_count_blocks(D, tiles) : 0;
+        if (count_blocks > 0) {
+            rc = launch_duplicate(*a, gs, gt, bt.tile_keys[0], bt.vals, (uint32_t)D, true, false, s);
+            if (rc != OGS_OK) return rc;
+            rc = launch_tile_count_binning(bt.tile_keys[0], bt.vals, D, n_dev, count_blocks, tiles, bt.tile_keys[1], is.ranges, bt.kept,
+                                           a->point_list, s, a->debug);
+            if (rc != OGS_OK) return rc;
+        } else {
+            const bool zero_in_dup = tiles <= (int64_t)a->P;
+            rc = launch_duplicate(*a, gs, gt, bt.tile_keys[0], vbuf[0], (uint32_t)D, cull, !per_tile, s,
+                                  zero_in_dup ? is.ranges : nullptr, zero_in_dup ? (int)tiles : 0);
+            if (rc != OGS_OK) return rc;
+            const bool sweep = radix_onesweep_enabled(D);
+            int shifts[4], nbits[4];
+            for (int p = 0; p < passes; ++p) {
+                shifts[p] = p * per;
+                nbits[p] = (p == passes - 1) ? (bits == 0 ? 1 : bits - shifts[p]) : per;
+            }
+            if (passes == 2 && (bits & 1)) {
+                nbits[0] = bits / 2; shifts[1] = nbits[0]; nbits[1] = bits - nbits[0];
+            }
+            if (sweep) {
+                rc = radix_sort_begin(bt.tile_keys[0], D, n_dev, passes, shifts, nbits, bt.sort_tmp, s, a->debug, cull);
+                if (rc != OGS_OK) return rc;
+            }
+            for (int p = 0; p < passes; ++p) {
+                const int in = p & 1, out = in ^ 1;
+                const bool drop = cull && p == 0;
+                const uint32_t* n_pass = (cull && p > 0) ? bt.kept : n_dev;
+                rc = sweep ? radix_sort_pass(p, passes, bt.tile_keys[in], vbuf[in], bt.tile_keys[out], vbuf[out], D, shifts[p], nbits[p], bt.sort_tmp, s, a->debug, n_pass, drop, drop ? bt.kept : nullptr)
+                           : radix_pass(bt.tile_keys[in], vbuf[in], bt.tile_keys[out], vbuf[out], D, shifts[p], nbits[p], bt.sort_tmp, s, a->debug, n_pass, drop, drop ? bt.kept : nullptr);
+                if (rc != OGS_OK) return rc;
+            }
+            rc = launch_tile_ranges(bt.tile_keys[passes & 1], D, is.ranges, tiles, s, a->debug, cull ? bt.kept : n_dev, zero_in_dup);
+            if (rc != OGS_OK) return rc;
         }
-        if (passes == 2 && (bits & 1)) {
-            nbits[0] = bits / 2; shifts[1] = nbits[0]; nbits[1] = bits - nbits[0];
-        }
-        if (sweep) {
-            rc = radix_sort_begin(bt.tile_keys[0], D, n_dev, passes, shifts, nbits, bt.sort_tmp, s, a->debug, cull);
-            if (rc != OGS_OK) return rc;
-        }
-        for (int p = 0; p < passes; ++p) {
-            const int in = p & 1, out = in ^ 1;
-            const bool drop = cull && p == 0;
-            const uint32_t* n_pass = (cull && p > 0) ? bt.kept : n_dev;
-            rc = sweep ? radix_sort_pass(p, passes, bt.tile_keys[in], vbuf[in], bt.tile_keys[out], vbuf[out], D, shifts[p], nbits[p], bt.sort_tmp, s, a->debug, n_pass, drop, drop ? bt.kept : nullptr)
-                       : radix_pass(bt.tile_keys[in], vbuf[in], bt.tile_keys[out], vbuf[out], D, shifts[p], nbits[p], bt.sort_tmp, s, a->debug, n_pass, drop, drop ? bt.kept : nullptr);
-            if (rc != OGS_OK) return rc;
-        }
-        rc = launch_tile_ranges(bt.tile_keys[passes & 1], D, is.ranges, tiles, s, a->debug, cull ? bt.kept : n_dev, zero_in_dup);
-        if (rc != OGS_OK) return rc;
         if (per_tile) {
             const uint32_t* order = launch_tile_order(is, tiles, a->P, s, a->debug);
             order_ready = true;
@@ -463,6 +472,12 @@
 size_t ogs_raster_tile_sort_capacity(int32_t level) {
     return level == 0 ? (size_t)kWaveSortCap : level == 1 ? (size_t)kTileSortCap : 0;
 }
+
+int ogs_raster_tile_count_debug(int64_t D, int64_t tiles, int32_t force_blocks, int32_t reverse) {
+    tile_count_debug(force_blocks, reverse);
+    return tile_count_blocks(D, tiles);
+}
+size_t ogs_raster_tile_count_trip(void) { return (size_t)tile_count_trip(); }
 
 static int forward_tiny_impl(const OgsRasterFwdArgs* a_in, void* stream_, bool raw, const float* raw_rest) {
     int rc = validate_fwd(a_in);
diff --git a/opengaussian_amd/csrc/ogs_common.h b/opengaussian_amd/csrc/ogs_common.h
--- a/opengaussian_amd/csrc/ogs_common.h
+++ b/opengaussian_amd/csrc/ogs_common.h
@@ -292,6 +292,13 @@
                      uint2* zero_ranges = nullptr, int n_zero = 0);
 int launch_tile_ranges(const uint32_t* tile_keys_sorted, int64_t D, uint2* ranges, int64_t tiles, hipStream_t s,
                        int debug, const uint32_t* n_dev = nullptr, bool already_zeroed = false);
+constexpr int kTileCountMaxTiles = 12288;
+constexpr int kTileCountBlocks = 128;
+int tile_count_blocks(int64_t D, int64_t tiles);
+int tile_count_trip();
+void tile_count_debug(int force_blocks, int reverse);
+int launch_tile_count_binning(const uint32_t* keys, const uint32_t* vals, int64_t D, const uint32_t* n_dev, int B, int64_t tiles,
+                              uint32_t* table, uint2* ranges, uint32_t* kept, uint32_t* point_list, hipStream_t s, int debug);
 inline bool per_tile_depth_order(const OgsRasterFwdArgs& a) { return a.num_groups <= 1 && a.P > kSmallMaxP; }
 inline bool block_sum_offsets(const OgsRasterFwdArgs& a) { return per_tile_depth_order(a) && a.full_binning == 0; }
 constexpr int kTileSortItems = 16;
```

After: 1547 Mpix/s, median of 6. 2.2% higher.
